# aelefebv/nellie

Hardware: AMD Instinct MI355X
Metric: Mvoxel/s multiscale Frangi (5 sigma) + Label, float32, frame resident in HBM (higher is better)
Workload: dtype f32; 1 GPU; synthetic 1024x1024x1024 float32 volume (N(100,5) noise + Gaussian tube segments, seed 2345), 0.1 um isotropic, 5-scale Frangi + Label, full hot path per step, frame resident in HBM; voxels=1073741824, labels=265, one_pass_scales=5, fast_div_proven=2, hessian_tile_rows=16

## Files before the change

nellie_amd/csrc/label_runs.inc:

```

struct RunRec { int row; unsigned int x; };
struct RunN { const unsigned int *p; i64 h; i64 cap; };
__device__ __forceinline__ i64 run_n(const RunN &r) { const i64 n = r.p ? (i64)*r.p : r.h; return n > r.cap ? 0 : n; }

__device__ __forceinline__ unsigned long long rl_word(const unsigned long long *__restrict__ bits, i64 row, int w, int wpr,
                                                      int nx, bool invert) {
    unsigned long long v = bits[row * wpr + w];
    if (invert) v = ~v;
    const int rem = nx - w * 64;
    if (rem < 64) v &= (rem <= 0) ? 0ull : ((1ull << rem) - 1ull);
    return v;
}

__global__ void __launch_bounds__(256)
rl_threshold_pack_kernel(const float *__restrict__ f, const unsigned long long *__restrict__ support, unsigned long long *__restrict__ bits,
                         int has_thr, float thr_host, int nx, i64 nrows, int wpr, const float *__restrict__ thr_dev = nullptr) {
    const float thr = thr_dev ? *thr_dev : thr_host;
    const i64 wstride = ((i64)gridDim.x * blockDim.x) >> 6;
    const int lane = threadIdx.x & 63;
    const bool row_words = support && wpr <= 64;
    const i64 first = ((i64)blockIdx.x * blockDim.x + threadIdx.x) >> 6;
    unsigned long long mine_next = (row_words && first < nrows && lane < wpr) ? support[first * wpr + lane] : 0ull;
    unsigned long long st_res = 0ull;
    i64 st_row = -1;
// ... 433 lines not shown
        const i64 i = base + k;
        if (i >= nruns) break;
        const int root = parent[i];
        const int len = (int)(runs[i].x >> 16) - (int)(runs[i].x & 0xffffu);
        unsigned int h = ((unsigned int)root * 2654435761u) >> 24;
        bool done = false;
        for (int probe = 0; probe < 8 && !done; ++probe) {
            const int old = atomicCAS(&keys[h], -1, root);
            if (old == -1 || old == root) { atomicAdd(&vals[h], len); done = true; }
            else h = (h + 1) & (RL_HT - 1);
        }
        if (!done) atomicAdd(&area[root], len);
    }
    __syncthreads();
    for (int k = threadIdx.x; k < RL_HT; k += 256)
        if (keys[k] >= 0 && vals[k]) atomicAdd(&area[keys[k]], vals[k]);
  }
}

__global__ void __launch_bounds__(256)
rl_keep_kernel(const RunRec *__restrict__ runs, const int *__restrict__ parent, const int *__restrict__ area, int min_area,
               unsigned long long *__restrict__ bits, RunN rn, int wpr) {
    const i64 nruns = run_n(rn);
    for (i64 i = (i64)blockIdx.x * blockDim.x + threadIdx.x; i < nruns; i += (i64)gridDim.x * blockDim.x) {
        if (area[parent[i]] < min_area) continue;
        const RunRec r = runs[i];
        rl_set_bits(bits, r.row, wpr, (int)(r.x & 0xffffu), (int)(r.x >> 16));
    }
}

__global__ void __launch_bounds__(256)
majority_bits_kernel(const unsigned long long *__restrict__ in, unsigned long long *__restrict__ out, VolGeom v, int wpr, i64 z_lo, i64 z_hi) {
    const unsigned int ny = (unsigned int)v.ny, uw = (unsigned int)wpr;
    const unsigned int nw = (unsigned int)(z_hi - z_lo) * ny * uw;
    const unsigned int t0 = blockIdx.x * blockDim.x + threadIdx.x;
    if (t0 >= nw) return;
    const unsigned int w = t0 % uw, row0 = t0 / uw;
    const int y = (int)(row0 % ny), z = (int)(row0 / ny) + (int)z_lo;
    const i64 t = ((i64)z * ny + y) * wpr + w;
    const bool last = (w == uw - 1u);
    const unsigned long long top = 1ull << (((int)v.nx - 1) & 63);
    const unsigned long long valid = (top << 1) - 1ull;
    unsigned long long c0 = 0, c1 = 0, c2 = 0, c3 = 0, c4 = 0;
    auto add = [&](unsigned long long b) {
        unsigned long long t0_ = c0 & b; c0 ^= b; b = t0_;
        t0_ = c1 & b; c1 ^= b; b = t0_;
        t0_ = c2 & b; c2 ^= b; b = t0_;
        t0_ = c3 & b; c3 ^= b; b = t0_;
        c4 ^= b;
    };
    unsigned long long cw[9];
    i64 rws[9];
    unsigned long long any = 0ull;
#pragma unroll
    for (int dz = -1; dz <= 1; ++dz) {
        int zz = z + dz;
        const i64 gg = v.gz0 + zz;
        if (gg < 0 || gg >= v.gnz) zz = z;
#pragma unroll
        for (int dy = -1; dy <= 1; ++dy) {
            int yy = y + dy;
            yy = yy < 0 ? 0 : (yy >= (int)ny ? (int)ny - 1 : yy);
            const int k = (dz + 1) * 3 + (dy + 1);
            rws[k] = ((i64)zz * ny + yy) * wpr;
            cw[k] = in[rws[k] + w];
            any |= cw[k];
        }
    }
    if (any == 0ull) { out[t] = 0ull; return; }
#pragma unroll
    for (int k = 0; k < 9; ++k) {
        const unsigned long long cur = cw[k];
        const unsigned long long prev = (w > 0u) ? in[rws[k] + w - 1] : 0ull;
        const unsigned long long left = (cur << 1) | ((w > 0u) ? (prev >> 63) : (cur & 1ull));
        const unsigned long long next = last ? 0ull : in[rws[k] + w + 1];
        const unsigned long long right = (cur >> 1) | (last ? (cur & top) : (next << 63));
        add(left); add(cur); add(right);
    }
    unsigned long long res = c4 | (c3 & c2 & c1);
    if (last) res &= valid;
    out[t] = res;
}

__global__ void __launch_bounds__(256)
rl_paint_kernel(const unsigned long long *__restrict__ bits, const unsigned int *__restrict__ row_off, const int *__restrict__ parent,
                const int *__restrict__ newid, int *__restrict__ out, i64 row0, i64 row1, int wpr, int nx) {
    const i64 wstride = ((i64)gridDim.x * blockDim.x) >> 6;
    const int lane = threadIdx.x & 63;
    for (i64 row = row0 + (((i64)blockIdx.x * blockDim.x + threadIdx.x) >> 6); row < row1; row += wstride) {
        const unsigned int seen0 = row_off[row], nr = row_off[row + 1] - seen0;
        unsigned int seen = seen0;
        int *orow = out + (row - row0) * nx;
        const bool vec = ((nx & 3) == 0) && ((reinterpret_cast<size_t>(orow) & 15) == 0);
        if (nr == 0u && vec) {
            for (int q = lane; q < nx / 4; q += 64) reinterpret_cast<int4 *>(orow)[q] = make_int4(0, 0, 0, 0);
            continue;
        }
        const int lab_mine = ((unsigned int)lane < nr) ? newid[parent[seen0 + lane]] : 0;
        if (vec) {
            for (int q = lane; q < nx / 4; q += 64) reinterpret_cast<int4 *>(orow)[q] = make_int4(0, 0, 0, 0);
            asm volatile("s_waitcnt vmcnt(0)" ::: "memory");
            unsigned long long carry = 0;
            int prev_w = -2;
            for (int wb = 0; wb < wpr; wb += 64) {
                const unsigned long long mine = (wb + lane < wpr) ? rl_word(bits, row, wb + lane, wpr, nx, false) : 0ull;
                unsigned long long todo = __ballot(mine != 0ull);
                while (todo) {
                    const int wl = __builtin_ctzll(todo);
                    todo &= todo - 1;
                    const int w = wb + wl;
                    const unsigned long long v = __shfl(mine, wl, 64);
                    if (w != prev_w + 1) carry = 0ull;
                    const unsigned long long starts = v & ~((v << 1) | carry);
                    const int x = w * 64 + lane;
                    const bool set = (v >> lane) & 1ull;
                    const unsigned long long below = starts & ((lane == 63) ? ~0ull : ((1ull << (lane + 1)) - 1ull));
                    const unsigned int rl = set ? (seen - seen0) + (unsigned int)__builtin_popcountll(below) - 1u : 0u;
                    int lab = __shfl(lab_mine, (int)(rl & 63u), 64);
                    if (set && rl >= 64u) lab = newid[parent[seen0 + rl]];
                    if (set && x < nx) orow[x] = lab;
                    seen += (unsigned int)__builtin_popcountll(starts);
                    carry = v >> 63;
                    prev_w = w;
                }
            }
            continue;
        }
        unsigned long long carry = 0;
        for (int wb = 0; wb < wpr; wb += 64) {
            const unsigned long long mine = (wb + lane < wpr) ? rl_word(bits, row, wb + lane, wpr, nx, false) : 0ull;
            const int wend = wpr - wb < 64 ? wpr - wb : 64;
            for (int wl = 0; wl < wend; ++wl) {
                const int w = wb + wl;
                const unsigned long long v = __shfl(mine, wl, 64);
                const unsigned long long starts = v & ~((v << 1) | carry);
                const int x = w * 64 + lane;
                const bool set = (v >> lane) & 1ull;
                const unsigned long long below = starts & ((lane == 63) ? ~0ull : ((1ull << (lane + 1)) - 1ull));
                const unsigned int rl = set ? (seen - seen0) + (unsigned int)__builtin_popcountll(below) - 1u : 0u;
                int lab = __shfl(lab_mine, (int)(rl & 63u), 64);
                if (set && rl >= 64u) lab = newid[parent[seen0 + rl]];
                if (x < nx) orow[x] = set ? lab : 0;
                seen += (unsigned int)__builtin_popcountll(starts);
                carry = v >> 63;
            }
        }
    }
}

#define SL_FILL 0
#define SL_AREA 1
#define SL_NUMBER 2

__global__ void __launch_bounds__(256)
sl_first_own_kernel(const RunRec *__restrict__ runs, const int *__restrict__ parent, int *__restrict__ aux, i64 nruns, int row_lo, int row_hi,
                    const unsigned int *__restrict__ own_first_ptr) {
    const i64 i = (i64)blockIdx.x * blockDim.x + threadIdx.x;
    if (i >= nruns) return;
    const int own_first = (int)*own_first_ptr;
    const int row = runs[i].row;
    if (row < row_lo || row >= row_hi) return;
    const int r = parent[i];
    if (r >= own_first) { if (r == (int)i) aux[i] = (int)i; return; }
    if ((int)i < __hip_atomic_load(&aux[r], __ATOMIC_RELAXED, __HIP_MEMORY_SCOPE_AGENT)) atomicMin(&aux[r], (int)i);
}
__global__ void __launch_bounds__(256)
sl_area_kernel(const RunRec *__restrict__ runs, const int *__restrict__ parent, int *__restrict__ area, i64 nruns, int row_lo, int row_hi) {
    __shared__ int keys[RL_HT];
    __shared__ int vals[RL_HT];
    for (int k = threadIdx.x; k < RL_HT; k += 256) { keys[k] = -1; vals[k] = 0; }
    __syncthreads();
    const i64 base = (i64)blockIdx.x * RL_CHUNK;
    for (int k = threadIdx.x; k < RL_CHUNK; k += 256) {
        const i64 i = base + k;
        if (i >= nruns) break;
        const RunRec r = runs[i];
        if (r.row < row_lo || r.row >= row_hi) continue;
        const int root = parent[i];
        const int len = (int)(r.x >> 16) - (int)(r.x & 0xffffu);
        unsigned int h = ((unsigned int)root * 2654435761u) >> 24;
        bool done = false;
        for (int probe = 0; probe < 8 && !done; ++probe) {
            const int old = atomicCAS(&keys[h], -1, root);
            if (old == -1 || old == root) { atomicAdd(&vals[h], len); done = true; }
            else h = (h + 1) & (RL_HT - 1);
        }
        if (!done) atomicAdd(&area[root], len);
    }
    __syncthreads();
    for (int k = threadIdx.x; k < RL_HT; k += 256)
        if (keys[k] >= 0 && vals[k]) atomicAdd(&area[keys[k]], vals[k]);
}
struct SlabPlanes { int row[4]; };
__global__ void __launch_bounds__(1024)
sl_boundary_kernel(const unsigned int *__restrict__ row_off, const int *__restrict__ proot, SlabPlanes pl, int ny, int capE,
                   int *__restrict__ bidx, int *__restrict__ hdr) {
    __shared__ unsigned int s_w[16];
    __shared__ unsigned int s_base;
    const int p = blockIdx.x;
    if (pl.row[p] < 0) { if (threadIdx.x == 0) hdr[p] = 0; return; }
    const unsigned int r0 = row_off[pl.row[p]], r1 = row_off[pl.row[p] + ny];
    const int lane = threadIdx.x & 63, w = threadIdx.x >> 6;
    if (threadIdx.x == 0) s_base = 0;
    __syncthreads();
    for (unsigned int c0 = r0; c0 < r1; c0 += 1024) {
        const unsigned int i = c0 + threadIdx.x;
        const bool f = i < r1 && (!proot || proot[i] == (int)i);
        const unsigned long long b = __ballot(f);
        const unsigned int below = (unsigned int)__builtin_popcountll(b & ((1ull << lane) - 1ull));
        if (lane == 0) s_w[w] = (unsigned int)__builtin_popcountll(b);
        __syncthreads();
        unsigned int off = s_base;
        for (int q = 0; q < w; ++q) off += s_w[q];
        if (f && off + below < (unsigned int)capE) bidx[(size_t)p * capE + off + below] = (int)i;
        __syncthreads();
        if (threadIdx.x == 0) { unsigned int t = 0; for (int q = 0; q < 16; ++q) t += s_w[q]; s_base += t; }
        __syncthreads();
    }
    if (threadIdx.x == 0) hdr[p] = (int)s_base;
}
__global__ void __launch_bounds__(256)
sl_table2_kernel(const int *__restrict__ parent, const int *__restrict__ aux, const uint8_t *__restrict__ flag, const int *__restrict__ bidx,
                 int capE, const int *__restrict__ hdr, int *__restrict__ blob, const unsigned int *__restrict__ nruns_ptr) {
    const int p = blockIdx.x;
    int cnt[4], total = 0, off = 8, over = 0;
// ... 63 lines not shown
```

nellie_amd/csrc/nellie_hip.hip:

```cpp
#include "nl_host.h"

struct RcclApi {
    void *handle = nullptr;
    decltype(&ncclGetUniqueId) GetUniqueId = nullptr;
    decltype(&ncclCommInitRank) CommInitRank = nullptr;
    decltype(&ncclCommDestroy) CommDestroy = nullptr;
    decltype(&ncclGetErrorString) GetErrorString = nullptr;
    decltype(&ncclGroupStart) GroupStart = nullptr;
    decltype(&ncclGroupEnd) GroupEnd = nullptr;
    decltype(&ncclSend) Send = nullptr;
    decltype(&ncclRecv) Recv = nullptr;
    decltype(&ncclAllReduce) AllReduce = nullptr;
    decltype(&ncclBroadcast) Broadcast = nullptr;
    decltype(&ncclAllGather) AllGather = nullptr;
    bool ok = false;
};
static RcclApi &rccl_real() {
    static RcclApi api;
    if (!api.handle) {
        std::string rp;
        if (const char *e = getenv("ROCM_PATH")) rp = std::string(e) + "/lib/librccl.so.1";
        const char *names[] = {rp.c_str(), "/opt/rocm/lib/librccl.so.1", "/opt/rocm/lib/librccl.so", "librccl.so.1", "librccl.so"};
        for (const char *n : names) { if (!*n) continue; api.handle = dlopen(n, RTLD_NOW | RTLD_GLOBAL); if (api.handle) break; }
        if (api.handle) {
// ... 327 lines not shown
    if (ok) ok = alloc((void **)&c->d_rows, ((size_t)nzl * ny + 2) * 2 * 4);
    if (ok) ok = alloc(&c->d_small, 1 << 16);
    c->vq_chunks = (int)vq_chunks(nzl, ny, nx);
    {
        const size_t qe = (size_t)vq_alloc_entries(nzl, ny, nx);
        if (ok) ok = alloc((void **)&c->d_vq, qe * 32);
        if (ok) ok = alloc((void **)&c->d_vq_count, (size_t)vq_alloc_regions(nzl, ny, nx) * 4);
        c->spec_ok = vq_spec_entries(nzl, ny, nx) > 0;
    }
    c->blk_cap = (n + SCAN_CHUNK - 1) / SCAN_CHUNK + 1;
    if (ok) ok = alloc(&c->d_blk, (size_t)c->blk_cap * 4);
    if (ok && hipHostMalloc(&c->h_small, 1 << 16, hipHostMallocDefault) != hipSuccess) {
        rc = nl_fail(err, errlen, NL_ENOMEM, "hipHostMalloc failed [out of memory]"); ok = false;
    }
    int side_prio = -1;
    { const char *e = getenv("NELLIE_SIDE_PRIO"); if (e) side_prio = atoi(e); }
    int prio_lo = 0, prio_hi = 0;
    (void)hipDeviceGetStreamPriorityRange(&prio_lo, &prio_hi);
    const int side_p = side_prio < 0 ? prio_hi : (side_prio > 0 ? prio_lo : (prio_lo + prio_hi) / 2);
    if (ok && (hipStreamCreateWithPriority(&c->side, hipStreamNonBlocking, side_p) != hipSuccess ||
               hipEventCreateWithFlags(&c->ev_side, hipEventDisableTiming) != hipSuccess ||
               hipEventCreateWithFlags(&c->ev_main, hipEventDisableTiming) != hipSuccess ||
               hipEventCreateWithFlags(&c->ev_ahead, hipEventDisableTiming) != hipSuccess)) {
        rc = nl_fail(err, errlen, NL_EHIP, "stream/event creation failed"); ok = false;
    }
    if (ok && (hipStreamCreateWithFlags(&c->stream, hipStreamNonBlocking) != hipSuccess ||
               hipEventCreate(&c->t0) != hipSuccess || hipEventCreate(&c->t1) != hipSuccess)) {
        rc = nl_fail(err, errlen, NL_EHIP, "stream/event creation failed"); ok = false;
    }
    if (!ok) { nl_ctx_destroy(c); return rc; }
    *out = c;
    return NL_OK;
}

extern "C" int nl_sync(nl_ctx *c, char *err, size_t errlen) {
    if (!c) return nl_fail(err, errlen, NL_EINVAL, "ctx is NULL");
    NL_HIP(hipSetDevice(c->device));
    NL_HIP(hipStreamSynchronize(c->stream));
    NL_HIP(hipStreamSynchronize(c->side));
    if (c->xstream) NL_HIP(hipStreamSynchronize(c->xstream));
    return NL_OK;
}


int upload_convert(nl_ctx *c, const void *host, int dtype, float *dst, i64 count, char *err, size_t errlen) {
    const size_t es = dtype_size(dtype);
    if (!es) return nl_fail(err, errlen, NL_EINVAL, "unsupported dtype code %d", dtype);
    if (dtype == NL_F32) {
        NL_HIP(hipMemcpyAsync(dst, host, (size_t)count * 4, hipMemcpyHostToDevice, c->stream));
        NL_HIP(hipStreamSynchronize(c->stream));
        return NL_OK;
    }
    void *raw = nullptr;
    bool own = false;
    for (int k = 0; k < 4 && !raw; ++k) {
        const bool contains = (dst >= c->f[k] && dst < c->f[k] + c->n);
        if (!contains && k != c->i_vmax && es <= 4) raw = c->f[k];
    }
    if (!raw) { NL_HIP(hipMalloc(&raw, (size_t)count * es)); own = true; }
    NL_HIP(hipMemcpyAsync(raw, host, (size_t)count * es, hipMemcpyHostToDevice, c->stream));
    const unsigned int g = grid1d(count);
    switch (dtype) {
        case NL_U8: convert_kernel<uint8_t><<<g, 256, 0, c->stream>>>((const uint8_t *)raw, dst, count); break;
        case NL_I8: convert_kernel<int8_t><<<g, 256, 0, c->stream>>>((const int8_t *)raw, dst, count); break;
        case NL_U16: convert_kernel<uint16_t><<<g, 256, 0, c->stream>>>((const uint16_t *)raw, dst, count); break;
        case NL_I16: convert_kernel<int16_t><<<g, 256, 0, c->stream>>>((const int16_t *)raw, dst, count); break;
        case NL_U32: convert_kernel<uint32_t><<<g, 256, 0, c->stream>>>((const uint32_t *)raw, dst, count); break;
        case NL_I32: convert_kernel<int32_t><<<g, 256, 0, c->stream>>>((const int32_t *)raw, dst, count); break;
        case NL_F64: convert_kernel<double><<<g, 256, 0, c->stream>>>((const double *)raw, dst, count); break;
        case NL_U64: convert_kernel<uint64_t><<<g, 256, 0, c->stream>>>((const uint64_t *)raw, dst, count); break;
        case NL_I64: convert_kernel<int64_t><<<g, 256, 0, c->stream>>>((const int64_t *)raw, dst, count); break;
    }
    NL_CHECK_LAUNCH();
    NL_HIP(hipStreamSynchronize(c->stream));
    if (own) hipFree(raw);
    return NL_OK;
}

extern "C" int nl_filter_load(nl_ctx *c, const void *host, int dtype, int64_t z0, int64_t z1, char *err, size_t errlen) {
    NL_ENTER(c);
    NL_JOIN_SIDE(c);
    if (!host || z0 < 0 || z1 > c->nzl || z0 >= z1) return nl_fail(err, errlen, NL_EINVAL, "bad plane range [%lld,%lld)", (i64)z0, (i64)z1);
    c->i_gauss = 0; c->i_vmax = 3; c->i_labels = -1; c->frangi_ready = 0;
    c->gauss_ext = nullptr;
    if (c->ahead_pending) NL_HIP(hipStreamWaitEvent(c->stream, c->ev_ahead, 0));
    c->ahead_pending = 0;
    c->fsq_cache_valid = 0;
    NL_HIP(zero_small((char *)c->d_small + (52 << 10), 4, c->stream));
    c->vmax_zero_lo = c->vmax_zero_hi = 0;
    const i64 plane = c->ny * c->nx;
    int rc = upload_convert(c, host, dtype, c->f[0] + z0 * plane, (z1 - z0) * plane, err, errlen);
    if (rc) return rc;
    c->mask_slots_used = 0;
    NL_HIP(hipStreamSynchronize(c->stream));
    return NL_OK;
}

extern "C" int nl_input_load(nl_ctx *c, const void *host, int dtype, int64_t z0, int64_t z1, char *err, size_t errlen) {
    NL_ENTER(c);
    const size_t es = dtype_size(dtype);
    if (!es) return nl_fail(err, errlen, NL_EINVAL, "unsupported dtype code %d", dtype);
    if (!host || z0 < 0 || z1 > c->nzl || z0 >= z1) return nl_fail(err, errlen, NL_EINVAL, "bad plane range [%lld,%lld)", (i64)z0, (i64)z1);
    if (c->d_input && c->input_borrowed) { c->d_input = nullptr; c->input_borrowed = 0; }
    if (c->d_input && c->input_dtype != dtype) { hipFree(c->d_input); c->d_input = nullptr; }
    if (!c->d_input) NL_HIP(hipMalloc(&c->d_input, (size_t)c->n * es));
    c->input_dtype = dtype;
    const i64 plane = c->ny * c->nx;
    NL_HIP(hipMemcpyAsync((char *)c->d_input + (size_t)z0 * plane * es, host, (size_t)(z1 - z0) * plane * es, hipMemcpyHostToDevice, c->stream));
    NL_HIP(hipStreamSynchronize(c->stream));
    return NL_OK;
}

extern "C" int nl_filter_begin(nl_ctx *c, char *err, size_t errlen) {
    NL_ENTER(c);
    NL_JOIN_SIDE(c);
    if (!c->d_input) return nl_fail(err, errlen, NL_ESTATE, "nl_filter_begin before nl_input_load");
    c->i_gauss = 0; c->i_vmax = 3; c->i_labels = -1; c->frangi_ready = 0;
    c->mask_slots_used = 0;
    c->gauss_ext = nullptr;
    if (c->ahead_pending) NL_HIP(hipStreamWaitEvent(c->stream, c->ev_ahead, 0));
    c->ahead_pending = 0;
    c->fsq_cache_valid = 0;
    NL_HIP(zero_small((char *)c->d_small + (52 << 10), 4, c->stream));
    c->vmax_zero_lo = c->vmax_zero_hi = 0;
    if (c->input_dtype == NL_F32 && !getenv("NELLIE_COPY_INPUT")) {
        c->gauss_ext = (float *)c->d_input;
        return NL_OK;
    }
    ProfScope ps(c, "load");
    const unsigned int g = grid1d(c->n);
    switch (c->input_dtype) {
        case NL_U8: convert_kernel<uint8_t><<<g, 256, 0, c->stream>>>((const uint8_t *)c->d_input, c->f[0], c->n); break;
        case NL_I8: convert_kernel<int8_t><<<g, 256, 0, c->stream>>>((const int8_t *)c->d_input, c->f[0], c->n); break;
        case NL_U16: convert_kernel<uint16_t><<<g, 256, 0, c->stream>>>((const uint16_t *)c->d_input, c->f[0], c->n); break;
        case NL_I16: convert_kernel<int16_t><<<g, 256, 0, c->stream>>>((const int16_t *)c->d_input, c->f[0], c->n); break;
        case NL_U32: convert_kernel<uint32_t><<<g, 256, 0, c->stream>>>((const uint32_t *)c->d_input, c->f[0], c->n); break;
        case NL_I32: convert_kernel<int32_t><<<g, 256, 0, c->stream>>>((const int32_t *)c->d_input, c->f[0], c->n); break;
        case NL_F32: convert_kernel<float><<<g, 256, 0, c->stream>>>((const float *)c->d_input, c->f[0], c->n); break;
        case NL_F64: convert_kernel<double><<<g, 256, 0, c->stream>>>((const double *)c->d_input, c->f[0], c->n); break;
        case NL_U64: convert_kernel<uint64_t><<<g, 256, 0, c->stream>>>((const uint64_t *)c->d_input, c->f[0], c->n); break;
        case NL_I64: convert_kernel<int64_t><<<g, 256, 0, c->stream>>>((const int64_t *)c->d_input, c->f[0], c->n); break;
    }
    NL_CHECK_LAUNCH();
    c->mask_slots_used = 0;
    return NL_OK;
}


static bool gauss_can_yx(const nl_ctx *c, const double *wy, int ry, const double *wx, int rx) {
    return wy && wx && ry == rx && ry >= 1 && ry <= GM_MAX_R && ry <= c->ny && !getenv("NELLIE_NO_FUSED_YX");
}
static int gauss_step_volumes(const nl_ctx *c, const double *wz, const double *wy, int ry, const double *wx, int rx) {
    return (wz ? 1 : 0) + (gauss_can_yx(c, wy, ry, wx, rx) ? 1 : (wy ? 1 : 0) + (wx ? 1 : 0));
}

extern "C" int nl_gauss_step(nl_ctx *c, const double *wz, int rz, const double *wy, int ry, const double *wx, int rx,
                             int64_t z0, int64_t z1, char *err, size_t errlen) {
    NL_ENTER(c);
    if (c->ahead_pending) return nl_fail(err, errlen, NL_ESTATE, "nl_gauss_step while a step enqueued ahead is uncommitted");
    if (z0 < 0 || z1 > c->nzl || z0 >= z1) return nl_fail(err, errlen, NL_EINVAL, "bad plane range [%lld,%lld)", (i64)z0, (i64)z1);
    if (c->halo_pending) {
        ProfScope ps(c, "halo_wait");
        NL_HIP(hipStreamWaitEvent(c->stream, c->ev_x_done, 0));
        c->halo_pending = 0;
    }
    const VolGeom v = geom(c);
    const dim3 grid((unsigned)((c->nx + 255) / 256), (unsigned)c->ny, (unsigned)(z1 - z0));
    int src = c->i_gauss;
    const float *srcp = gauss_cur(c);
    GaussW gw;
    int rc;
    const bool can_yx = gauss_can_yx(c, wy, ry, wx, rx);
    bool fused_yx = false;
    const char *e_fz = getenv("NELLIE_GAUSS_FUSED");
    const bool fused_zyx = e_fz ? atoi(e_fz) != 0 : c->n >= ((i64)1 << 26);
    if (fused_zyx && wz && can_yx && gyx_tiled() && gl_zyx_ok(c, rz, ry, c->f[(src + 1) % 3]) &&
        memcmp(wy, wx, (size_t)(2 * ry + 1) * sizeof(double)) == 0) {
        GaussW gy;
        if ((rc = fill_gw(gw, wz, rz, err, errlen)) || (rc = fill_gw(gy, wy, ry, err, errlen))) return rc;
        if ((z0 - rz < 0 && c->gz0 > 0) || (z1 - 1 + rz >= c->nzl && c->gz0 + c->nzl < c->gnz))
            return nl_fail(err, errlen, NL_EINVAL, "Z pass of radius %d on planes [%lld,%lld) reaches outside the local slab", rz, (i64)z0, (i64)z1);
        const int dst = (src + 1) % 3;
        char scope[32];
        snprintf(scope, sizeof scope, "gauss_zyx<%d,%d>", rz, ry);
        ProfScope ps(c, scope);
        static int zero_in_passing = -1;
        if (zero_in_passing < 0) { const char *e = getenv("NELLIE_ZERO_IN_GAUSS"); zero_in_passing = (e && !atoi(e)) ? 0 : 1; }
        const bool zero = zero_in_passing && c->mask_slots_used == 0 && c->vmax_zero_hi == 0 && c->stream != c->side;
        (void)gl_zyx(c, rz, ry, srcp, c->f[dst], v, z0, z1, gauss_ws_of(gw), gauss_ws_of(gy), zero ? c->f[c->i_vmax] : nullptr);
        if (zero) { c->vmax_zero_lo = z0; c->vmax_zero_hi = z1; }
        NL_CHECK_LAUNCH();
        src = dst; srcp = c->f[dst];
        fused_yx = true;
        wz = nullptr;
    }
    if (wz) {
        if ((rc = fill_gw(gw, wz, rz, err, errlen))) return rc;
        if ((z0 - rz < 0 && c->gz0 > 0) || (z1 - 1 + rz >= c->nzl && c->gz0 + c->nzl < c->gnz))
            return nl_fail(err, errlen, NL_EINVAL, "Z pass of radius %d on planes [%lld,%lld) reaches outside the local slab", rz, (i64)z0, (i64)z1);
        const int dst = (src + 1) % 3;
        ProfScope ps(c, "gauss_z");
        if (!gl_fast(0, c, srcp, c->f[dst], v, z0, z1, gw)) gl_axis(0, false, c, grid, srcp, c->f[dst], v, z0, z1, gw);
        NL_CHECK_LAUNCH();
        src = dst; srcp = c->f[dst];
    }
    if (!fused_yx && can_yx) {
        GaussW gy, gx;
        if ((rc = fill_gw(gy, wy, ry, err, errlen))) return rc;
        if ((rc = fill_gw(gx, wx, rx, err, errlen))) return rc;
        const GaussWS wsy = gauss_ws_of(gy), wsx = gauss_ws_of(gx);
        const int dst = (src + 1) % 3;
        ProfScope ps(c, "gauss_yx");
        const dim3 g2((unsigned)((c->nx + GYX_COLS - 1) / GYX_COLS), (unsigned)((c->ny + v.chunk - 1) / v.chunk), (unsigned)(z1 - z0));
        (void)gl_yx(c, gyx_tiled(), false, ry, srcp, c->f[dst], v, z0, z1, wsy, wsx, g2);
        NL_CHECK_LAUNCH();
        src = dst; srcp = c->f[dst];
        fused_yx = true;
    }
    if (wy && !fused_yx) {
        if ((rc = fill_gw(gw, wy, ry, err, errlen))) return rc;
        const int dst = (src + 1) % 3;
        ProfScope ps(c, "gauss_y");
        if (!gl_fast(1, c, srcp, c->f[dst], v, z0, z1, gw)) gl_axis(1, false, c, grid, srcp, c->f[dst], v, z0, z1, gw);
        NL_CHECK_LAUNCH();
        src = dst; srcp = c->f[dst];
    }
    if (wx && !fused_yx) {
        if ((rc = fill_gw(gw, wx, rx, err, errlen))) return rc;
        const int dst = (src + 1) % 3;
        ProfScope ps(c, "gauss_x");
        if (!gl_fast(2, c, srcp, c->f[dst], v, z0, z1, gw)) gl_axis(2, false, c, grid, srcp, c->f[dst], v, z0, z1, gw);
        NL_CHECK_LAUNCH();
        src = dst; srcp = c->f[dst];
    }
    c->i_gauss = src;
    c->fsq_cache_valid = 0;
    if (srcp != c->gauss_ext) c->gauss_ext = nullptr;
    return NL_OK;
}

extern "C" int nl_gauss_step_ahead(nl_ctx *c, const double *wz, int rz, const double *wy, int ry, const double *wx, int rx,
                                   int64_t z0, int64_t z1, char *err, size_t errlen) {
    NL_ENTER(c);
    if (c->ahead_pending) return nl_fail(err, errlen, NL_ESTATE, "a step enqueued ahead is already pending");
    if (gauss_step_volumes(c, wz, wy, ry, wx, rx) > 2)
        return nl_fail(err, errlen, NL_ESTATE, "a cascade step of three passes (radii %d / %d / %d) cannot run ahead: it needs the current Gaussian's volume", rz, ry, rx);
    NL_HIP(hipEventRecord(c->ev_main, c->stream));
    hipStream_t ahead_stream = c->side;
    NL_HIP(hipStreamWaitEvent(ahead_stream, c->ev_main, 0));
    const int cur_idx = c->i_gauss;
    float *cur_ext = c->gauss_ext;
    hipStream_t main_stream = c->stream;
    c->stream = ahead_stream;
    const int rc = nl_gauss_step(c, wz, rz, wy, ry, wx, rx, z0, z1, err, errlen);
    c->stream = main_stream;
    if (rc) { c->i_gauss = cur_idx; c->gauss_ext = cur_ext; return rc; }
    c->ahead_gauss = c->i_gauss;
    c->i_gauss = cur_idx; c->gauss_ext = cur_ext;
    NL_HIP(hipEventRecord(c->ev_ahead, ahead_stream));
    c->ahead_pending = 1;
    return NL_OK;
}

extern "C" int nl_gauss_commit(nl_ctx *c, char *err, size_t errlen) {
    NL_ENTER(c);
    if (!c->ahead_pending) return nl_fail(err, errlen, NL_ESTATE, "nl_gauss_commit without nl_gauss_step_ahead");
    NL_HIP(hipStreamWaitEvent(c->stream, c->ev_ahead, 0));
    c->i_gauss = c->ahead_gauss;
    c->gauss_ext = nullptr;
    c->ahead_pending = 0;
    c->fsq_cache_valid = 0;
    return NL_OK;
}

static int make_lattice(const nl_ctx *c, i64 sz, i64 sy, i64 sx, Lattice &L, char *err, size_t errlen) {
    if (sz < 1 || sy < 1 || sx < 1) return nl_fail(err, errlen, NL_EINVAL, "strides must be >= 1");
    L.sz = sz; L.sy = sy; L.sx = sx;
    const i64 g_lo = c->gz0 + c->own_lo, g_hi = c->gz0 + c->own_hi;
    const i64 k_lo = (g_lo + sz - 1) / sz, k_hi = (g_hi + sz - 1) / sz;
    L.cz = k_hi > k_lo ? k_hi - k_lo : 0;
    L.zfirst = k_lo * sz - c->gz0;
    L.cy = (c->ny + sy - 1) / sy;
    L.cx = (c->nx + sx - 1) / sx;
    return NL_OK;
}

static int make_field(nl_ctx *c, int field, FieldSrc &fs, char *err, size_t errlen) {
    fs.field = field; fs.hp = hessp(c); fs.max_abs = c->frob_max_abs; fs.max_finite = c->frob_max_finite;
    fs.two_d = c->two_d; fs.bits = nullptr; fs.wpr = 0; fs.fsq_cache = nullptr; fs.norm_dev = nullptr;
    if (field == NL_FIELD_GAUSS) fs.p = gauss_cur(c);
    else if (field == NL_FIELD_FROB) {
        if (!c->have_spacing) return nl_fail(err, errlen, NL_ESTATE, "NL_FIELD_FROB before nl_hessian_stats");
        fs.p = gauss_cur(c);
    } else if (field == NL_FIELD_FRANGI) fs.p = c->f[c->i_vmax];
    else if (field == NL_FIELD_VESSELNESS) {
        if (c->mask_slots_used == 0) return nl_fail(err, errlen, NL_ESTATE, "NL_FIELD_VESSELNESS before any scale was evaluated");
        NL_JOIN_SIDE(c);
        fs.p = c->f[c->i_vmax];
        fs.wpr = (int)((c->nx + 63) / 64);
        fs.bits = (const unsigned long long *)c->m[0] + (i64)((c->mask_slots_used - 1) & 1) * (c->nzl * c->ny * fs.wpr);
    } else return nl_fail(err, errlen, NL_EINVAL, "unknown field %d", field);
    return NL_OK;
}

static int use_fsq_cache(nl_ctx *c, FieldSrc &fs, const Lattice &L, char *err, size_t errlen) {
    if (fs.field != NL_FIELD_FROB) return NL_OK;
    const i64 total = L.cz * L.cy * L.cx;
    if (total == 0) return NL_OK;
    if (!(c->fsq_cache_valid && c->fsq_cache_key[0] == L.sz && c->fsq_cache_key[1] == L.sy && c->fsq_cache_key[2] == L.sx)) {
        if (total > c->fsq_cache_cap) {
            if (c->d_fsq_cache) NL_HIP(hipFree(c->d_fsq_cache));
            c->d_fsq_cache = nullptr; c->fsq_cache_cap = 0;
            NL_HIP(hipMalloc((void **)&c->d_fsq_cache, (size_t)total * 4));
            c->fsq_cache_cap = total;
        }
        ProfScope ps(c, "sample");
        sample_fsq_kernel<<<(unsigned)((total + 255) / 256), 256, 0, c->stream>>>(fs, geom(c), L, c->d_fsq_cache);
        NL_CHECK_LAUNCH();
        c->fsq_cache_key[0] = L.sz; c->fsq_cache_key[1] = L.sy; c->fsq_cache_key[2] = L.sx;
        c->fsq_cache_valid = 1;
    }
    fs.fsq_cache = c->d_fsq_cache;
    return NL_OK;
}

extern "C" int nl_sample_gather(nl_ctx *c, int field, int64_t sz, int64_t sy, int64_t sx, float *out, int64_t cap,
                                int64_t *n, char *err, size_t errlen) {
    NL_ENTER(c);
    Lattice L; FieldSrc fs; int rc;
    if ((rc = make_lattice(c, sz, sy, sx, L, err, errlen))) return rc;
    if ((rc = make_field(c, field, fs, err, errlen))) return rc;
    if ((rc = use_fsq_cache(c, fs, L, err, errlen))) return rc;
    const i64 total = L.cz * L.cy * L.cx;
    if (n) *n = total;
    if (total == 0 || (!out && cap == 0)) return NL_OK;
    if (!out || cap < total) return nl_fail(err, errlen, NL_EINVAL, "output capacity %lld < %lld samples", (i64)cap, total);
    float *stage = c->f[(c->i_gauss + 1) % 3];
    if (total > c->n) return nl_fail(err, errlen, NL_EINVAL, "lattice larger than the volume");
    {
        ProfScope ps(c, "sample");
        sample_gather_kernel<<<(unsigned)((total + 255) / 256), 256, 0, c->stream>>>(fs, geom(c), L, stage);
        NL_CHECK_LAUNCH();
    }
    NL_HIP(hipMemcpyAsync(out, stage, (size_t)total * 4, hipMemcpyDeviceToHost, c->stream));
    NL_HIP(hipStreamSynchronize(c->stream));
    return NL_OK;
}

// ... 631 lines not shown
    { int rc = resolve_enqueue(c, vp, d_cnt, nullptr, err, errlen); if (rc) return rc; }
    *hit = 1;
    if (mask_count) {
        int rcc = nl_vesselness_count(c, mask_count, err, errlen);
        if (rcc) return rcc;
    }
    return NL_OK;
}


static void host_edges(float first, float last, int nbins, float *edges) {
    if (first == last) { first = first - 0.5f; last = last + 0.5f; }
    volatile float delta = last - first;
    const float div = (float)nbins;
    volatile float step = delta / div;
    for (int i = 0; i <= nbins; ++i) {
        volatile float y = (float)i;
        if (step == 0.0f) { y = y / div; y = y * delta; } else y = y * step;
        y = y + first;
        edges[i] = (i == nbins) ? last : y;
    }
}
static inline unsigned int f2u(float x) { unsigned int u; memcpy(&u, &x, 4); return u; }
static inline float u2f(unsigned int u) { float x; memcpy(&x, &u, 4); return x; }
static inline float py_min_f(float a, float b) { return b < a ? b : a; }

static int chain_verify(const ChainScale &s, double division, double margin, double test_scale) {
    if (s.flags) return s.flags;
    int bad = 0;
    double tri, otsu; int st;
    {
        hist_thresholds_host<float>((const int64_t *)s.h_gauss.counts, s.h_gauss.edges, NL_CHAIN_BINS, &tri, &otsu, &st);
        const float g = py_min_f((float)tri, (float)otsu);
        const float gamma = g > 0.0f ? g : 1.1920929e-07f;
        const float gamma_sq = (float)(2.0 * std::pow((double)gamma, 2.0));
        if (st || f2u(gamma) != f2u(s.gamma) || f2u(gamma_sq) != f2u(s.gamma_sq)) bad = 1;
        float e[NL_CHAIN_BINS + 1];
        host_edges(u2f(s.h_gauss.res[0]), u2f(s.h_gauss.res[1]), NL_CHAIN_BINS, e);
        if (memcmp(e, s.h_gauss.edges, sizeof(e))) bad = 1;
    }
    {
        hist_thresholds_host<float>((const int64_t *)s.h_raw.counts, s.h_raw.edges, NL_CHAIN_BINS, &tri, &otsu, &st);
        const double t = (double)py_min_f((float)tri, (float)otsu) * test_scale / division;
        const float lo = (float)(t * t * (1.0 - margin)), hi = (float)(t * t * (1.0 + margin));
        if (st || f2u(lo) != f2u(s.fsq_lo) || f2u(hi) != f2u(s.fsq_hi)) bad = 1;
        float e[NL_CHAIN_BINS + 1];
        host_edges(u2f(s.h_raw.res[0]), u2f(s.h_raw.res[1]), NL_CHAIN_BINS, e);
        if (memcmp(e, s.h_raw.edges, sizeof(e))) bad = 1;
    }
    {
        const float max_abs32 = u2f(s.stats[0]), max_fsq32 = u2f(s.stats[1]);
        const float max_abs = max_abs32 <= 0.0f ? 1.0f : max_abs32;
        volatile float mf = sqrtf(max_fsq32); mf = mf / max_abs;
        volatile float mn = u2f(s.h_raw.res[0]) / max_abs, mx = u2f(s.h_raw.res[1]) / max_abs;
        if (f2u(max_abs) != f2u(s.max_abs) || f2u((float)mf) != f2u(s.max_frob) || f2u((float)mn) != f2u(s.nmn) || f2u((float)mx) != f2u(s.nmx) ||
            f2u(s.norm[0]) != f2u(max_abs) || s.norm[1] != 0.0f) bad = 1;
        float e[NL_CHAIN_BINS + 1];
        host_edges((float)mn, (float)mx, NL_CHAIN_BINS, e);
        if (memcmp(e, s.h_exact.edges, sizeof(e))) bad = 1;
        hist_thresholds_host<float>((const int64_t *)s.h_exact.counts, s.h_exact.edges, NL_CHAIN_BINS, &tri, &otsu, &st);
        const float thr = py_min_f((float)tri, (float)otsu);
        const float thr_cmp = (float)((double)thr / division);
        const float fsq_min = mask_threshold_on_fsq(max_abs, 1, thr_cmp);
        if (st || f2u(thr) != f2u(s.thr) || f2u(thr_cmp) != f2u(s.thr_cmp) || f2u(fsq_min) != f2u(s.fsq_min) || s.m_inf != ((0.0f > thr_cmp) ? 1 : 0)) bad = 1;
        if (!(fsq_min >= s.fsq_lo && fsq_min <= s.fsq_hi) || !((float)mf > thr_cmp)) bad = 1;
    }
    return bad ? NL_CF_VERIFY : 0;
}

extern "C" int nl_chain_begin(nl_ctx *c, int n_scales, char *err, size_t errlen) {
    NL_ENTER(c);
    if (n_scales < 1 || n_scales > NL_CHAIN_MAX_SCALES) return nl_fail(err, errlen, NL_EINVAL, "a chain holds 1..%d scales", NL_CHAIN_MAX_SCALES);
    if (!c->two_d && (!c->spec_ok || !hv_rs(c))) return nl_fail(err, errlen, NL_ESTATE, "the device-resident chain needs the 3-D one-pass walk");
    if (!c->d_chain) {
        NL_HIP(hipMalloc(&c->d_chain, sizeof(ChainScale) * NL_CHAIN_MAX_SCALES));
        NL_HIP(hipHostMalloc(&c->h_chain, sizeof(ChainScale) * NL_CHAIN_MAX_SCALES, hipHostMallocDefault));
        NL_HIP(hipEventCreateWithFlags(&c->ev_chain, hipEventDisableTiming));
    }
    chain_init_kernel<<<16, 256, 0, c->stream>>>((ChainScale *)c->d_chain, n_scales);
    chain_init2_kernel<<<1, 64, 0, c->stream>>>((ChainScale *)c->d_chain, n_scales);
    NL_CHECK_LAUNCH();
    c->chain_n = n_scales; c->chain_k = 0; c->chain_copy_pending = 0;
    c->def_resolve = 0;
    return NL_OK;
}

extern "C" int nl_chain_scale(nl_ctx *c, const double spacing[3], int64_t sz, int64_t sy, int64_t sx, double alpha_sq, double beta_sq,
                              double division, double margin, double test_scale, int64_t z0, int64_t z1, char *err, size_t errlen) {
    NL_ENTER(c);
    if (!c->d_chain || c->chain_k >= c->chain_n) return nl_fail(err, errlen, NL_ESTATE, "nl_chain_scale outside nl_chain_begin .. nl_chain_finish");
    if (!(division != 0.0)) return nl_fail(err, errlen, NL_EINVAL, "the chain needs a non-zero threshold division");
    int rc;
    if ((rc = set_spacing(c, spacing, err, errlen))) return rc;
    if ((rc = resolve_deferred_launch(c, true, err, errlen))) return rc;
    ChainScale *cs = (ChainScale *)c->d_chain + c->chain_k;
    c->chain_par[c->chain_k][0] = division; c->chain_par[c->chain_k][1] = margin; c->chain_par[c->chain_k][2] = test_scale;
    ++c->chain_k;
    c->frob_max_abs = 1.0f; c->frob_max_finite = 0.0f;
    if (c->two_d) {
        if (!chain_unfused_sampling()) {
            if ((rc = range_hist_pair_enqueue(c, sz, sy, sx, NL_CHAIN_BINS, (char *)&cs->h_gauss, (char *)&cs->h_raw, nullptr, nullptr, err, errlen))) return rc;
        } else {
            if ((rc = range_hist_enqueue_at(c, NL_FIELD_GAUSS, sz, sy, sx, NL_CHAIN_BINS, (char *)&cs->h_gauss, nullptr, err, errlen))) return rc;
            if ((rc = range_hist_enqueue_at(c, NL_FIELD_FROB, sz, sy, sx, NL_CHAIN_BINS, (char *)&cs->h_raw, nullptr, err, errlen))) return rc;
        }
        chain_thr1_kernel<<<2, 64, 0, c->stream>>>(cs, division, margin, test_scale);
        {
            ProfScope ps(c, "hessian_stats");
            hessian2d_stats_kernel<<<grid2d_rows(c->nx, c->ny), 256, 0, c->stream>>>(gauss_cur(c), geom(c), hessp(c), cs->stats);
        }
        chain_post_kernel<<<1, 64, 0, c->stream>>>(cs);
        NL_CHECK_LAUNCH();
        {
            Lattice L; FieldSrc fs;
            if ((rc = make_lattice(c, sz, sy, sx, L, err, errlen))) return rc;
            if ((rc = make_field(c, NL_FIELD_FROB, fs, err, errlen))) return rc;
            if ((rc = use_fsq_cache(c, fs, L, err, errlen))) return rc;
            fs.norm_dev = cs->norm;
            const i64 total = L.cz * L.cy * L.cx;
            ProfScope ps(c, "sample");
            sample_edges_kernel<<<1, 64, 0, c->stream>>>(cs->h_exact.res, NL_CHAIN_BINS, cs->h_exact.edges, cs->h_exact.res + 4);
            const size_t sh = (size_t)(NL_CHAIN_BINS + 2) * 4 + (size_t)NL_CHAIN_BINS * 4;
            if (total > 0) sample_hist_kernel<<<grid1d(total, 256, sample_grid_cap()), 256, sh, c->stream>>>(fs, geom(c), L, cs->h_exact.edges, NL_CHAIN_BINS, cs->h_exact.counts, cs->h_exact.res + 4);
            NL_CHECK_LAUNCH();
        }
        chain_thr2_kernel<<<1, 64, 0, c->stream>>>(cs, division);
        NL_CHECK_LAUNCH();
        VessP vp{};
        vp.alpha_sq = (float)alpha_sq; vp.beta_sq = (float)beta_sq; vp.use_thr = 1;
        vp.cnt_lo = (int)c->own_lo; vp.cnt_hi = (int)c->own_hi;
        vp.first = c->mask_slots_used == 0 ? 1 : 0;
        vp.nan_flag = (unsigned int *)((char *)c->d_small + NL_NAN_FLAG_OFF);
        ProfScope ps(c, "vesselness");
        const int wpr = (int)((c->nx + 63) / 64);
        const i64 slot_words = c->nzl * c->ny * wpr;
        const int k_scale = c->mask_slots_used++;
        vp.have_prev = k_scale > 0;
        unsigned long long *cm = (unsigned long long *)c->m[0] + (i64)(k_scale & 1) * slot_words;
        const unsigned long long *pm = (unsigned long long *)c->m[0] + (i64)((k_scale + 1) & 1) * slot_words;
        if (vp.first && !vmax_is_zero(c, 0, c->nzl)) NL_HIP(hipMemsetAsync(c->f[c->i_vmax], 0, (size_t)c->n * 4, c->stream));
        c->vmax_zero_hi = 0;
        c->spec_valid = 0;
        vesselness2d_kernel<<<grid2d_rows((i64)wpr * 64, c->ny), 256, 0, c->stream>>>(gauss_cur(c), c->f[c->i_vmax], cm, pm, wpr, geom(c), hessp(c), vp,
                                                                                        &cs->cnt_resolve, (const float *)cs);
        NL_CHECK_LAUNCH();
        return NL_OK;
    }
    if (!chain_unfused_sampling()) {
        if ((rc = range_hist_pair_enqueue(c, sz, sy, sx, NL_CHAIN_BINS, (char *)&cs->h_gauss, (char *)&cs->h_raw, nullptr, nullptr, err, errlen))) return rc;
    } else {
        if ((rc = range_hist_enqueue_at(c, NL_FIELD_GAUSS, sz, sy, sx, NL_CHAIN_BINS, (char *)&cs->h_gauss, nullptr, err, errlen))) return rc;
        if ((rc = range_hist_enqueue_at(c, NL_FIELD_FROB, sz, sy, sx, NL_CHAIN_BINS, (char *)&cs->h_raw, nullptr, err, errlen))) return rc;
    }
    chain_thr1_kernel<<<2, 64, 0, c->stream>>>(cs, division, margin, test_scale);
    NL_CHECK_LAUNCH();
    if ((rc = spec_enqueue(c, spacing, 0.0f, 0.0f, z0, z1, cs->stats, &cs->cnt_walk, &cs->fsq_lo, err, errlen))) return rc;
    const bool defer = resolve_defer_ok(c) && c->fsq_cache_valid;
    hipStream_t st = c->stream;
    chain_post_kernel<<<1, 64, 0, st>>>(cs);
    NL_CHECK_LAUNCH();
    {
        Lattice L; FieldSrc fs;
        if ((rc = make_lattice(c, sz, sy, sx, L, err, errlen))) return rc;
        if ((rc = make_field(c, NL_FIELD_FROB, fs, err, errlen))) return rc;
        if ((rc = use_fsq_cache(c, fs, L, err, errlen))) return rc;
        fs.norm_dev = cs->norm;
        const i64 total = L.cz * L.cy * L.cx;
        ProfScope ps(c, "sample", st);
        sample_edges_kernel<<<1, 64, 0, st>>>(cs->h_exact.res, NL_CHAIN_BINS, cs->h_exact.edges, cs->h_exact.res + 4);
        const size_t sh = (size_t)(NL_CHAIN_BINS + 2) * 4 + (size_t)NL_CHAIN_BINS * 4;
        if (total > 0) sample_hist_kernel<<<grid1d(total, 256, sample_grid_cap()), 256, sh, st>>>(fs, geom(c), L, cs->h_exact.edges, NL_CHAIN_BINS, cs->h_exact.counts, cs->h_exact.res + 4);
        NL_CHECK_LAUNCH();
        if (fused(c) && (rc = reduce_u64_sum(c, cs->h_exact.counts, NL_CHAIN_BINS, err, errlen))) return rc;
    }
    chain_thr2_kernel<<<1, 64, 0, st>>>(cs, division);
    NL_CHECK_LAUNCH();
    VessP vp{};
    vp.alpha_sq = (float)alpha_sq; vp.beta_sq = (float)beta_sq; vp.use_thr = 1;
    vp.cnt_lo = (int)c->own_lo; vp.cnt_hi = (int)c->own_hi;
    vp.first = c->mask_slots_used == 0 ? 1 : 0;
    if (defer) {
        memcpy(c->def_vp, &vp, sizeof(VessP));
        c->def_cnt = &cs->cnt_resolve; c->def_params = (const float *)cs; c->def_resolve = 1;
        return NL_OK;
    }
    return resolve_enqueue(c, vp, &cs->cnt_resolve, (const float *)cs, err, errlen);
}

extern "C" int nl_chain_flush(nl_ctx *c, char *err, size_t errlen) {
    NL_ENTER(c);
    if (!c->d_chain || c->chain_k < 1) return nl_fail(err, errlen, NL_ESTATE, "nl_chain_flush without scales");
    { int rcd = resolve_deferred_launch(c, false, err, errlen); if (rcd) return rcd; }
    NL_JOIN_SIDE(c);
    NL_HIP(hipMemcpyAsync(c->h_chain, c->d_chain, sizeof(ChainScale) * (size_t)c->chain_k, hipMemcpyDeviceToHost, c->stream));
    NL_HIP(hipEventRecord(c->ev_chain, c->stream));
    c->chain_copy_pending = 1;
    return NL_OK;
}

extern "C" int nl_chain_finish(nl_ctx *c, int *flags, double *gamma, double *max_abs, double *thr, int64_t *mask_count, char *err, size_t errlen) {
    NL_ENTER(c);
    if (!c->d_chain || c->chain_k < 1) return nl_fail(err, errlen, NL_ESTATE, "nl_chain_finish without scales");
    const int n = c->chain_k;
    if (!c->chain_copy_pending) { int rcd = resolve_deferred_launch(c, false, err, errlen); if (rcd) return rcd; }
    if (c->chain_copy_pending) {
        NL_HIP(hipEventSynchronize(c->ev_chain));
        c->chain_copy_pending = 0;
    } else {
        NL_JOIN_SIDE(c);
        NL_HIP(hipMemcpyAsync(c->h_chain, c->d_chain, sizeof(ChainScale) * (size_t)n, hipMemcpyDeviceToHost, c->stream));
        NL_HIP(hipStreamSynchronize(c->stream));
    }
    const ChainScale *h = (const ChainScale *)c->h_chain;
    for (int k = 0; k < n; ++k) {
        const int f = chain_verify(h[k], c->chain_par[k][0], c->chain_par[k][1], c->chain_par[k][2]);
        if (flags) flags[k] = f;
        if (gamma) gamma[k] = (double)h[k].gamma;
        if (max_abs) max_abs[k] = (double)h[k].max_abs;
        if (thr) thr[k] = (double)h[k].thr;
        if (mask_count) mask_count[k] = (int64_t)(h[k].cnt_walk + h[k].cnt_resolve);
    }
    c->chain_n = 0;
    return NL_OK;
}

extern "C" int nl_chain_log(nl_ctx *c, int k, int which, int64_t *counts, float *edges, float *range, double *scalars, char *err, size_t errlen) {
    if (!c || !c->h_chain || k < 0 || k >= NL_CHAIN_MAX_SCALES || which < 0 || which > 2) return nl_fail(err, errlen, NL_EINVAL, "bad chain log request");
    const ChainScale &s = ((const ChainScale *)c->h_chain)[k];
    const ChainHist &h = which == 0 ? s.h_gauss : (which == 1 ? s.h_raw : s.h_exact);
    if (counts) memcpy(counts, h.counts, sizeof(h.counts));
    if (edges) memcpy(edges, h.edges, sizeof(h.edges));
    if (range) { range[0] = u2f(h.res[0]); range[1] = u2f(h.res[1]); }
    if (scalars) {
        scalars[0] = s.fsq_lo; scalars[1] = s.fsq_hi; scalars[2] = s.gamma_sq; scalars[3] = s.fsq_min; scalars[4] = s.thr_cmp; scalars[5] = s.max_frob;
        scalars[6] = s.tri[which]; scalars[7] = s.otsu[which];
    }
    return NL_OK;
}

extern "C" int nl_vesselness_step(nl_ctx *c, float gamma_sq, float alpha_sq, float beta_sq, int use_thr, float thr,
                                  int64_t z0, int64_t z1, int64_t *mask_count, char *err, size_t errlen) {
    NL_ENTER(c);
    if (z0 < 0 && z1 < 0) { z0 = c->own_lo; z1 = c->own_hi; }
    if (z0 < 0 || z1 > c->nzl || z0 >= z1) return nl_fail(err, errlen, NL_EINVAL, "bad plane range [%lld,%lld)", (i64)z0, (i64)z1);
    if (!c->have_spacing) return nl_fail(err, errlen, NL_ESTATE, "nl_vesselness_step before nl_hessian_stats");
    NL_JOIN_SIDE(c);
    unsigned long long *d_cnt = (unsigned long long *)c->d_small;
    NL_HIP(zero_small(d_cnt, 8, c->stream));
    VessP vp = make_vessp(c, gamma_sq, alpha_sq, beta_sq, use_thr, thr);
    vp.qcap = HM_REGION;
    c->spec_valid = 0;
    if (c->two_d) {
        ProfScope ps(c, "vesselness");
        const int wpr = (int)((c->nx + 63) / 64);
        const i64 slot_words = c->nzl * c->ny * wpr;
        const int k_scale = c->mask_slots_used++;
        vp.have_prev = k_scale > 0;
        unsigned long long *cm = (unsigned long long *)c->m[0] + (i64)(k_scale & 1) * slot_words;
        const unsigned long long *pm = (unsigned long long *)c->m[0] + (i64)((k_scale + 1) & 1) * slot_words;
        if (vp.first && !vmax_is_zero(c, 0, c->nzl)) NL_HIP(hipMemsetAsync(c->f[c->i_vmax], 0, (size_t)c->n * 4, c->stream));
        c->vmax_zero_hi = 0;
        vesselness2d_kernel<<<grid2d_rows((i64)wpr * 64, c->ny), 256, 0, c->stream>>>(gauss_cur(c), c->f[c->i_vmax], cm, pm, wpr, geom(c), hessp(c), vp, d_cnt);
        NL_CHECK_LAUNCH();
    } else {
        ProfScope ps(c, "vesselness");
        const int ntx = (int)((c->nx + HM_TX - 1) / HM_TX);
        const int wpr = (int)((c->nx + 63) / 64);
        const i64 slot_words = c->nzl * c->ny * wpr;
        const int k_scale = c->mask_slots_used++;
        vp.have_prev = k_scale > 0;
        unsigned long long *cm = (unsigned long long *)c->m[0] + (i64)(k_scale & 1) * slot_words;
        const unsigned long long *pm = (unsigned long long *)c->m[0] + (i64)((k_scale + 1) & 1) * slot_words;
        const i64 plane = c->ny * c->nx;
        const i64 planes_per_launch = (i64)c->vq_chunks * HM_ZCHUNK;
        const VQueue vq{(float4 *)c->d_vq, c->d_vq_count};
        if (vp.first && !vmax_is_zero(c, z0, z1))
            NL_HIP(hipMemsetAsync(c->f[c->i_vmax] + z0 * plane, 0, (size_t)(z1 - z0) * plane * 4, c->stream));
        c->vmax_zero_hi = 0;
        const int rs = hv_rs(c);
        const int ty = rs ? 2 * rs : hm_ty();
        const int nty = (int)((c->ny + ty - 1) / ty);
        if (rs) vp.qcap = 2 * hv_np(c) * HM_REGION;
#define NL_LAUNCH_VESS(TYV, FASTV, HR)                                                                                    \
        hessian_g_kernel<1, TYV, FASTV><<<nblocks, HGCfg<TYV>::NT, HGCfg<TYV>::lds_bytes(), c->stream>>>(                 \
            gauss_cur(c), cm, pm, wpr, geom(c), HR, vp, vq, (int)za, (int)zb, ntx, nty, nullptr, d_cnt)
        for (i64 za = z0; za < z1; za += planes_per_launch) {
            const i64 zb = za + planes_per_launch < z1 ? za + planes_per_launch : z1;
            const int nzc = (int)((zb - za + HM_ZCHUNK - 1) / HM_ZCHUNK);
            const unsigned nblocks = (unsigned)(ntx * nty * nzc);
            if (rs) NL_HIP(nl_hv_launch(HvLaunch{1, rs, hv_np(c), hv_fastv(c), nblocks, c->stream, gauss_cur(c), cm, pm, wpr, geom(c), hessp(c), vp, vq, (int)za, (int)zb,
                                                 ntx, nty, nullptr, d_cnt, nullptr}));
            else if (ty == 8) { if (c->fast_div) NL_LAUNCH_VESS(8, true, hessdv_fast(c)); else NL_LAUNCH_VESS(8, false, hessdv_exact(c)); }
            else { if (c->fast_div) NL_LAUNCH_VESS(16, true, hessdv_fast(c)); else NL_LAUNCH_VESS(16, false, hessdv_exact(c)); }
            NL_CHECK_LAUNCH();
            const unsigned nregions = nblocks * (unsigned)(rs ? rs / hv_np(c) : ty);
            vesselness_queue_kernel<false><<<resolve_grid((nregions + 3) / 4), 256, 0, c->stream>>>(vq.ent, vq.count, nregions, c->f[c->i_vmax], za * plane, vp,
                                                                                      nullptr, nullptr, wpr, (int)c->ny, (int)c->nx, za, nullptr, nullptr);
            NL_CHECK_LAUNCH();
        }
#undef NL_LAUNCH_VESS
        NL_CHECK_LAUNCH();
    }
    if (mask_count) {
        NL_HIP(hipMemcpyAsync(c->h_small, d_cnt, 8, hipMemcpyDeviceToHost, c->stream));
        NL_HIP(hipStreamSynchronize(c->stream));
// ... 76 lines not shown
    if (z0 < 0 && z1 < 0) { z0 = c->own_lo; z1 = c->own_hi; }
    if (z0 < 0 || z1 > c->nzl || z0 >= z1) return nl_fail(err, errlen, NL_EINVAL, "bad plane range [%lld,%lld)", (i64)z0, (i64)z1);
    NL_JOIN_SIDE(c);
    unsigned long long *d_cnt = (unsigned long long *)c->d_small;
    NL_HIP(zero_small(d_cnt, 8, c->stream));
    const i64 plane = c->ny * c->nx;
    if (c->mask_slots_used == 0 && !vmax_is_zero(c, z0, z1))
        NL_HIP(hipMemsetAsync(c->f[c->i_vmax] + z0 * plane, 0, (size_t)(z1 - z0) * plane * 4, c->stream));
    c->vmax_zero_hi = 0;
    {
        ProfScope ps(c, "finish");
        const int wpr = (int)((c->nx + 63) / 64);
        const i64 quads = (z1 - z0) * c->ny * ((c->nx + 3) / 4);
        const i64 slot_words = c->nzl * c->ny * wpr;
        const int last = c->mask_slots_used > 0 ? ((c->mask_slots_used - 1) & 1) : 0;
        finish_kernel<<<grid1d(quads, 256, 256 * 16), 256, 0, c->stream>>>(c->f[c->i_vmax], (const unsigned long long *)c->m[0] + last * slot_words,
                                                               c->mask_slots_used > 0 ? 1 : 0, slot_words, wpr, geom(c), z0, z1, c->own_lo, c->own_hi, d_cnt);
        NL_CHECK_LAUNCH();
    }
    NL_HIP(hipMemcpyAsync(c->h_small, d_cnt, 8, hipMemcpyDeviceToHost, c->stream));
    NL_HIP(hipStreamSynchronize(c->stream));
    if (n_positive) *n_positive = (int64_t)(*(unsigned long long *)c->h_small);
    c->frangi_ready = 1;
    return NL_OK;
}

extern "C" int nl_remove_edges(nl_ctx *c, int margin, int64_t *n_positive, char *err, size_t errlen) {
    NL_ENTER(c);
    NL_JOIN_SIDE(c);
    if (!c->frangi_ready) return nl_fail(err, errlen, NL_ESTATE, "nl_remove_edges before a Frangi frame exists");
    if (margin < 0) return nl_fail(err, errlen, NL_EINVAL, "margin %d is negative", margin);
    unsigned long long *d_cnt = (unsigned long long *)c->d_small;
    NL_HIP(zero_small(d_cnt, 8, c->stream));
    {
        ProfScope ps(c, "finish");
        const i64 r0 = c->own_lo - 2 > 0 ? c->own_lo - 2 : 0, r1 = c->own_hi + 2 < c->nzl ? c->own_hi + 2 : c->nzl;
        remove_edges_kernel<<<(unsigned)(r1 - r0), 256, 0, c->stream>>>(c->f[c->i_vmax], geom(c), r0, margin, c->own_lo, c->own_hi, d_cnt);
        NL_CHECK_LAUNCH();
    }
    NL_HIP(hipMemcpyAsync(c->h_small, d_cnt, 8, hipMemcpyDeviceToHost, c->stream));
    NL_HIP(hipStreamSynchronize(c->stream));
    if (n_positive) *n_positive = (int64_t)(*(unsigned long long *)c->h_small);
    return NL_OK;
}

static int mask_volume_enqueue(nl_ctx *c, float thr, const float *thr_dev, int *dst_out, char *err, size_t errlen) {
    int dst = -1;
    for (int k = 0; k < 3; ++k) if (k != c->i_gauss) { dst = k; break; }
    *dst_out = dst;
    ProfScope ps(c, "mask_volume");
    const int wpr = (int)((c->nx + 63) / 64);
    const VolGeom v = geom(c);
    const i64 m0 = c->own_lo - 2 > 0 ? c->own_lo - 2 : 0, m1 = c->own_hi + 2 < c->nzl ? c->own_hi + 2 : c->nzl;
    const i64 e0 = c->own_lo - 1 > 0 ? c->own_lo - 1 : 0, e1 = c->own_hi + 1 < c->nzl ? c->own_hi + 1 : c->nzl;
    unsigned long long *bM = (unsigned long long *)c->m[1], *bE = (unsigned long long *)c->m[2], *bD = (unsigned long long *)c->m[0];
    nl_launch_threshold_pack(grid1d((m1 - m0) * c->ny * 64, 256, (i64)1 << 22), c->stream,
        c->f[c->i_vmax] + m0 * c->ny * c->nx, nullptr, bM + m0 * c->ny * wpr, 1, thr, (int)c->nx, (m1 - m0) * c->ny, wpr, thr_dev);
    NL_CHECK_LAUNCH();
    bits_morph6_kernel<0><<<(unsigned)(((e1 - e0) * c->ny * wpr + 255) / 256), 256, 0, c->stream>>>(bM, bE, v, wpr, e0, e1, c->two_d);
    NL_CHECK_LAUNCH();
    bits_morph6_kernel<1><<<(unsigned)(((c->own_hi - c->own_lo) * c->ny * wpr + 255) / 256), 256, 0, c->stream>>>(bE, bD, v, wpr, c->own_lo, c->own_hi, c->two_d);
    NL_CHECK_LAUNCH();
    apply_bits_kernel<<<grid1d((c->own_hi - c->own_lo) * c->ny * ((c->nx + 3) / 4), 256, 256 * 32), 256, 0, c->stream>>>(
        c->f[c->i_vmax], bD, c->f[dst], v, wpr, c->own_lo, c->own_hi);
    NL_CHECK_LAUNCH();
    return NL_OK;
}
static void mask_volume_commit(nl_ctx *c, int dst) {
    float *tmp = c->f[c->i_vmax];
    c->f[c->i_vmax] = c->f[dst];
    c->f[dst] = tmp;
}

extern "C" int nl_mask_volume(nl_ctx *c, float thr, char *err, size_t errlen) {
    NL_ENTER(c);
    int dst, rc;
    if ((rc = mask_volume_enqueue(c, thr, nullptr, &dst, err, errlen))) return rc;
    mask_volume_commit(c, dst);
    return NL_OK;
}

static int mask_volume_fused_enqueue(nl_ctx *c, float thr, const float *thr_dev, unsigned long long *d_cnt, int *dst_out, char *err, size_t errlen) {
    int dst = -1;
    for (int k = 0; k < 3; ++k) if (k != c->i_gauss) { dst = k; break; }
    *dst_out = dst;
    NL_HIP(zero_small(d_cnt, 8, c->stream));
    ProfScope ps(c, "mask_volume");
    const int wpr = (int)((c->nx + 63) / 64);
    const VolGeom v = geom(c);
    const i64 slot_words = c->nzl * c->ny * wpr;
    const int last = (c->mask_slots_used - 1) & 1;
    const unsigned long long *alive = (const unsigned long long *)c->m[0] + (i64)last * slot_words;
    const i64 m0 = c->own_lo - 2 > 0 ? c->own_lo - 2 : 0, m1 = c->own_hi + 2 < c->nzl ? c->own_hi + 2 : c->nzl;
    const i64 e0 = c->own_lo - 1 > 0 ? c->own_lo - 1 : 0, e1 = c->own_hi + 1 < c->nzl ? c->own_hi + 1 : c->nzl;
    unsigned long long *bM = (unsigned long long *)c->m[1], *bE = (unsigned long long *)c->m[2];
    unsigned long long *bD = (unsigned long long *)c->m[0] + (i64)(last ^ 1) * slot_words;
    pack_masked_kernel<<<grid1d((m1 - m0) * c->ny * 64, 256, 256 * 16), 256, 0, c->stream>>>(
        c->f[c->i_vmax], alive, bM, thr, thr_dev, (int)c->nx, m0 * c->ny, m1 * c->ny, wpr, c->own_lo * c->ny, c->own_hi * c->ny, d_cnt);
    NL_CHECK_LAUNCH();
    bits_morph6_kernel<0><<<(unsigned)(((e1 - e0) * c->ny * wpr + 255) / 256), 256, 0, c->stream>>>(bM, bE, v, wpr, e0, e1, c->two_d);
    NL_CHECK_LAUNCH();
    bits_morph6_kernel<1><<<(unsigned)(((c->own_hi - c->own_lo) * c->ny * wpr + 255) / 256), 256, 0, c->stream>>>(bE, bD, v, wpr, c->own_lo, c->own_hi, c->two_d);
    NL_CHECK_LAUNCH();
    apply_bits_pos_kernel<<<grid1d(((c->own_hi - c->own_lo) * c->ny + APPLY_ROWS - 1) / APPLY_ROWS * 64, 256, (i64)1 << 22), 256, 0, c->stream>>>(
        c->f[c->i_vmax], bD, c->f[dst], v, wpr, c->own_lo, c->own_hi);
    NL_CHECK_LAUNCH();
    if (fused(c)) NL_NCCL(rccl().AllReduce(d_cnt, d_cnt, 1, ncclUint64, ncclSum, (ncclComm_t)c->comm, c->stream));
    return NL_OK;
}
static void mask_volume_fused_commit(nl_ctx *c, int dst) {
    float *tmp = c->f[c->i_vmax];
    c->f[c->i_vmax] = c->f[dst];
    c->f[dst] = tmp;
    c->frangi_ready = 1;
    c->d_support = (const unsigned long long *)c->m[0] + (i64)(((c->mask_slots_used - 1) & 1) ^ 1) * (c->nzl * c->ny * (i64)((c->nx + 63) / 64));
    c->support_epoch = c->epoch.load();
}

extern "C" int nl_mask_volume_fused(nl_ctx *c, float thr, int64_t *n_positive, char *err, size_t errlen) {
    NL_ENTER(c);
    if (c->mask_slots_used == 0) return nl_fail(err, errlen, NL_ESTATE, "nl_mask_volume_fused before any scale was evaluated");
    NL_JOIN_SIDE(c);
    unsigned long long *d_cnt = (unsigned long long *)c->d_small;
    int dst, rc;
    if ((rc = mask_volume_fused_enqueue(c, thr, nullptr, d_cnt, &dst, err, errlen))) return rc;
    NL_HIP(hipMemcpyAsync(c->h_small, d_cnt, 8, hipMemcpyDeviceToHost, c->stream));
    NL_HIP(hipStreamSynchronize(c->stream));
    if (n_positive) *n_positive = (int64_t)(*(unsigned long long *)c->h_small);
    mask_volume_fused_commit(c, dst);
    return NL_OK;
}

static int pct_buffers(nl_ctx *c, char *err, size_t errlen) {
    if (!c->d_pct) {
        NL_HIP(hipMalloc(&c->d_pct, 128 + (size_t)2 * PCT_BINS * 4));
        NL_HIP(hipHostMalloc(&c->h_pct, 128, hipHostMallocDefault));
    }
    return NL_OK;
}
static int pct_enqueue(nl_ctx *c, const float *samples, const unsigned int *d_n, i64 max_n, float q, char *err, size_t errlen) {
    PctRec *rec = (PctRec *)c->d_pct;
    unsigned int *hist = (unsigned int *)((char *)c->d_pct + 128);
    NL_HIP(hipMemcpyAsync(&rec->n, d_n, 4, hipMemcpyDeviceToDevice, c->stream));
    NL_HIP(hipMemcpyAsync(&rec->n_local, d_n, 4, hipMemcpyDeviceToDevice, c->stream));
    if (fused(c)) NL_NCCL(rccl().AllReduce(&rec->n, &rec->n, 1, ncclUint32, ncclSum, (ncclComm_t)c->comm, c->stream));
    ProfScope ps(c, "sample");
    pct_begin_kernel<<<1, 64, 0, c->stream>>>(rec, q);
    const unsigned grid = grid1d(max_n > 0 ? max_n : 1, 256, 256 * 256);
#define NL_PCT_LEVEL(L)                                                                                            \
    NL_HIP(hipMemsetAsync(hist, 0, (size_t)2 * PCT_BINS * 4, c->stream));                                           \
    pct_hist_kernel<L><<<grid, 256, 0, c->stream>>>(samples, d_n, rec, hist);                                       \
    if (fused(c)) NL_NCCL(rccl().AllReduce(hist, hist, (size_t)2 * PCT_BINS, ncclUint32, ncclSum, (ncclComm_t)c->comm, c->stream)); \
    pct_select_kernel<L><<<1, 256, 0, c->stream>>>(rec, hist);
    NL_PCT_LEVEL(0) NL_PCT_LEVEL(1) NL_PCT_LEVEL(2)
#undef NL_PCT_LEVEL
    NL_CHECK_LAUNCH();
    return NL_OK;
}

extern "C" int nl_tail_enqueue(nl_ctx *c, int64_t sz, int64_t sy, int64_t sx, double q, char *err, size_t errlen) {
    NL_ENTER(c);
    if (c->mask_slots_used == 0) return nl_fail(err, errlen, NL_ESTATE, "nl_tail_enqueue before any scale was evaluated");
    if (c->two_d) return nl_fail(err, errlen, NL_EINVAL, "nl_tail_enqueue is the 3-D epilogue");
    int rc;
    if ((rc = pct_buffers(c, err, errlen))) return rc;
    Lattice L; FieldSrc fs;
    if ((rc = make_lattice(c, sz, sy, sx, L, err, errlen))) return rc;
    if ((rc = make_field(c, NL_FIELD_VESSELNESS, fs, err, errlen))) return rc;
    const i64 total = L.cz * L.cy * L.cx;
    if (total > c->n) return nl_fail(err, errlen, NL_EINVAL, "lattice larger than the volume");
    float *stage = c->f[(c->i_gauss + 1) % 3];
    if (stage == c->f[c->i_vmax]) return nl_fail(err, errlen, NL_ESTATE, "no free volume for the samples");
    unsigned int *d_n = (unsigned int *)((char *)c->d_pct + 64);
    unsigned long long *d_cnt = (unsigned long long *)((char *)c->d_pct + 72);
    NL_HIP(zero_small(d_n, 4, c->stream));
    if (total > 0) {
        ProfScope ps(c, "sample");
        sample_gather_pos_kernel<<<(unsigned)((total + 255) / 256), 256, 0, c->stream>>>(fs, geom(c), L, stage, d_n);
        NL_CHECK_LAUNCH();
    }
    if ((rc = pct_enqueue(c, stage, d_n, total, (float)q, err, errlen))) return rc;
    int dst;
    if ((rc = mask_volume_fused_enqueue(c, 0.0f, &((PctRec *)c->d_pct)->thr, d_cnt, &dst, err, errlen))) return rc;
    NL_HIP(hipMemcpyAsync(c->h_pct, c->d_pct, 80, hipMemcpyDeviceToHost, c->stream));
    c->tail_pending = 1; c->tail_dst = dst;
    return NL_OK;
}

extern "C" int nl_tail_finish(nl_ctx *c, int commit, int64_t *n_samples, float *a, float *b, float *gamma, float *thr, int64_t *n_positive,
                              char *err, size_t errlen) {
    NL_ENTER(c);
    if (!c->tail_pending) return nl_fail(err, errlen, NL_ESTATE, "nl_tail_finish without nl_tail_enqueue");
    NL_HIP(hipStreamSynchronize(c->stream));
    c->tail_pending = 0;
    const PctRec *rec = (const PctRec *)c->h_pct;
    if (n_samples) *n_samples = rec->n;
    if (a) *a = rec->a;
    if (b) *b = rec->b;
    if (gamma) *gamma = rec->gamma;
    if (thr) *thr = rec->thr;
    if (n_positive) *n_positive = (int64_t)(*(const unsigned long long *)((const char *)c->h_pct + 72));
    if (commit && rec->n > 0) mask_volume_fused_commit(c, c->tail_dst);
    return NL_OK;
}

extern "C" int nl_mask_volume_dev(nl_ctx *c, int64_t sz, int64_t sy, int64_t sx, double q, int64_t *n_samples, float *a, float *b, float *gamma,
                                  float *thr, char *err, size_t errlen) {
    NL_ENTER(c);
    int rc;
    if ((rc = pct_buffers(c, err, errlen))) return rc;
    Lattice L; FieldSrc fs;
    if ((rc = make_lattice(c, sz, sy, sx, L, err, errlen))) return rc;
    if ((rc = make_field(c, NL_FIELD_FRANGI, fs, err, errlen))) return rc;
    const i64 total = L.cz * L.cy * L.cx;
    if (total > c->n) return nl_fail(err, errlen, NL_EINVAL, "lattice larger than the volume");
    float *stage = nullptr;
    for (int k = 0; k < 3; ++k) if (k != c->i_gauss && c->f[k] != c->f[c->i_vmax]) stage = c->f[k];
    if (!stage) return nl_fail(err, errlen, NL_ESTATE, "no free volume for the samples");
    unsigned int *d_n = (unsigned int *)((char *)c->d_pct + 64);
    NL_HIP(zero_small(d_n, 4, c->stream));
    if (total > 0) {
        ProfScope ps(c, "sample");
        sample_gather_pos_kernel<<<(unsigned)((total + 255) / 256), 256, 0, c->stream>>>(fs, geom(c), L, stage, d_n);
        NL_CHECK_LAUNCH();
    }
    if ((rc = pct_enqueue(c, stage, d_n, total, (float)q, err, errlen))) return rc;
    int dst;
    if ((rc = mask_volume_enqueue(c, 0.0f, &((PctRec *)c->d_pct)->thr, &dst, err, errlen))) return rc;
    NL_HIP(hipMemcpyAsync(c->h_pct, c->d_pct, 64, hipMemcpyDeviceToHost, c->stream));
    NL_HIP(hipStreamSynchronize(c->stream));
    const PctRec *rec = (const PctRec *)c->h_pct;
    if (n_samples) *n_samples = rec->n;
    if (a) *a = rec->a;
    if (b) *b = rec->b;
    if (gamma) *gamma = rec->gamma;
    if (thr) *thr = rec->thr;
    if (rec->n > 0) mask_volume_commit(c, dst);
    return NL_OK;
}

extern "C" int nl_debug_percentile(nl_ctx *c, const float *values, int64_t n, double q, float *thr, float *a, float *b, char *err, size_t errlen) {
    NL_ENTER(c);
    if (!values || n < 1 || n > c->n) return nl_fail(err, errlen, NL_EINVAL, "bad sample array");
    int rc;
    if ((rc = pct_buffers(c, err, errlen))) return rc;
    float *stage = c->f[(c->i_gauss + 1) % 3];
    unsigned int *d_n = (unsigned int *)((char *)c->d_pct + 64);
    const unsigned int un = (unsigned int)n;
    NL_HIP(hipMemcpyAsync(stage, values, (size_t)n * 4, hipMemcpyHostToDevice, c->stream));
    NL_HIP(hipMemcpyAsync(d_n, &un, 4, hipMemcpyHostToDevice, c->stream));
    NL_HIP(hipStreamSynchronize(c->stream));
    const int keep = c->fuse_reduce; c->fuse_reduce = 0;
    rc = pct_enqueue(c, stage, d_n, n, (float)q, err, errlen);
    c->fuse_reduce = keep;
    if (rc) return rc;
    NL_HIP(hipMemcpyAsync(c->h_pct, c->d_pct, 64, hipMemcpyDeviceToHost, c->stream));
    NL_HIP(hipStreamSynchronize(c->stream));
    const PctRec *rec = (const PctRec *)c->h_pct;
    if (thr) *thr = rec->thr;
    if (a) *a = rec->a;
    if (b) *b = rec->b;
    return NL_OK;
}

int store_planes(nl_ctx *c, const void *dev_base, void *host, size_t elem, int64_t z0, int64_t z1, char *err, size_t errlen) {
    if (!host || z0 < 0 || z1 > c->nzl || z0 >= z1) return nl_fail(err, errlen, NL_EINVAL, "bad plane range [%lld,%lld)", (i64)z0, (i64)z1);
    const i64 plane = c->ny * c->nx;
    NL_HIP(hipMemcpyAsync(host, (const char *)dev_base + (size_t)z0 * plane * elem, (size_t)(z1 - z0) * plane * elem,
                          hipMemcpyDeviceToHost, c->stream));
    NL_HIP(hipStreamSynchronize(c->stream));
    return NL_OK;
}

extern "C" int nl_filter_store(nl_ctx *c, float *host, int64_t z0, int64_t z1, char *err, size_t errlen) {
    NL_ENTER(c);
    NL_KEEP_LABBITS(c);
    NL_KEEP_SUPPORT(c);
    return store_planes(c, c->f[c->i_vmax], host, 4, z0, z1, err, errlen);
}
extern "C" int nl_gauss_store(nl_ctx *c, float *host, int64_t z0, int64_t z1, char *err, size_t errlen) {
    NL_ENTER(c);
    return store_planes(c, gauss_cur(c), host, 4, z0, z1, err, errlen);
}

static float *field_ptr(nl_ctx *c, int field) {
    if (field == NL_FIELD_GAUSS) return gauss_cur(c);
    if (field == NL_FIELD_FRANGI) return c->f[c->i_vmax];
    return nullptr;
}

extern "C" int nl_planes_get(nl_ctx *c, int field, int64_t z0, int64_t z1, float *host, char *err, size_t errlen) {
    NL_ENTER(c);
    float *p = field_ptr(c, field);
    if (!p) return nl_fail(err, errlen, NL_EINVAL, "nl_planes_get: field %d has no volume", field);
    return store_planes(c, p, host, 4, z0, z1, err, errlen);
}

extern "C" int nl_planes_put(nl_ctx *c, int field, int64_t z0, int64_t z1, const float *host, char *err, size_t errlen) {
    NL_ENTER(c);
    float *p = field_ptr(c, field);
    c->fsq_cache_valid = 0;
    if (!p || !host || z0 < 0 || z1 > c->nzl || z0 >= z1) return nl_fail(err, errlen, NL_EINVAL, "nl_planes_put: bad field or plane range");
    const i64 plane = c->ny * c->nx;
    NL_HIP(hipMemcpyAsync(p + z0 * plane, host, (size_t)(z1 - z0) * plane * 4, hipMemcpyHostToDevice, c->stream));
    NL_HIP(hipStreamSynchronize(c->stream));
    return NL_OK;
}


extern "C" int nl_comm_unique_id(char *id128, char *err, size_t errlen) {
    if (!id128) return nl_fail(err, errlen, NL_EINVAL, "id buffer is NULL");
    ncclUniqueId id;
    {
        (void)hipGetLastError();
        ncclResult_t r_ = rccl().GetUniqueId(&id);
        if (r_ != ncclSuccess) return nl_fail(err, errlen, NL_ECOMM, "ncclGetUniqueId: %s", rccl().GetErrorString(r_));
    }
    static_assert(sizeof(id) == 128, "ncclUniqueId is 128 bytes");
    memcpy(id128, &id, 128);
    return NL_OK;
}

extern "C" int nl_comm_loopback_id(char *id128, char *err, size_t errlen) {
    if (!id128) return nl_fail(err, errlen, NL_EINVAL, "id buffer is NULL");
    lb::get_unique_id(id128);
    return NL_OK;
}

struct PooledComm { int device, world, rank, role; ncclComm_t comm; };
static std::mutex g_comm_pool_mu;
static std::vector<PooledComm> g_comm_pool;
static ncclComm_t comm_pool_take(int device, int world, int rank, int role) {
    std::lock_guard<std::mutex> lk(g_comm_pool_mu);
    for (size_t i = 0; i < g_comm_pool.size(); ++i) {
        const PooledComm &p = g_comm_pool[i];
        if (p.device == device && p.world == world && p.rank == rank && p.role == role) {
            ncclComm_t c = p.comm;
            g_comm_pool.erase(g_comm_pool.begin() + (long)i);
            return c;
        }
    }
    return nullptr;
}
static void comm_release(nl_ctx *c, void *comm, int role) {
    if (!comm) return;
    if (lb::is_ours(comm) || c->comm_poisoned || getenv("NELLIE_DESTROY_COMMS")) { rccl().CommDestroy((ncclComm_t)comm); return; }
    std::lock_guard<std::mutex> lk(g_comm_pool_mu);
    g_comm_pool.push_back(PooledComm{c->device, c->world, c->rank, role, (ncclComm_t)comm});
}
static int comm_acquire(nl_ctx *c, int world, int rank, const char *id128, int role, ncclComm_t *out, char *err, size_t errlen) {
    ncclUniqueId id;
    memcpy(&id, id128, 128);
    if (!lb::is_loopback_id(id128)) {
        ncclComm_t pooled = comm_pool_take(c->device, world, rank, role);
        if (pooled) { *out = pooled; return NL_OK; }
    }
    (void)hipGetLastError();
    NL_NCCL(rccl().CommInitRank(out, world, id, rank));
// ... 159 lines not shown
    const float *h = (const float *)c->h_ag;
    for (int r = 0; r < W; ++r) {
        unsigned int k; memcpy(&k, h + (size_t)r * blk, 4);
        if ((i64)k > block_items) return nl_fail(err, errlen, NL_ESTATE, "rank %d reports %u samples in a block of %lld", r, k, (long long)block_items);
        counts[r] = (int64_t)k;
        if (total + (i64)k > cap || (k && !out)) return nl_fail(err, errlen, NL_EINVAL, "output capacity %lld too small", (long long)cap);
        if (k) memcpy(out + total, h + (size_t)r * blk + 1, (size_t)k * 4);
        total += (i64)k;
    }
    return NL_OK;
}

extern "C" int nl_allgather_bytes(nl_ctx *c, const void *send, int64_t nbytes, void *recv, int64_t max_bytes, int64_t *bytes_of,
                                  char *err, size_t errlen) {
    NL_ENTER(c);
    NL_KEEP_SUPPORT(c);
    if (!c->comm) return nl_fail(err, errlen, NL_ESTATE, "nl_allgather_bytes before nl_comm_init");
    if (nbytes < 0 || max_bytes < 1 || nbytes > max_bytes || !recv || !bytes_of || (nbytes && !send))
        return nl_fail(err, errlen, NL_EINVAL, "bad all-gather arguments");
    const int W = c->world;
    long long *hs = (long long *)c->h_small;
    hs[0] = nbytes;
    NL_HIP(hipMemcpyAsync(c->d_small, hs, 8, hipMemcpyHostToDevice, c->stream));
    NL_NCCL(rccl().AllGather(c->d_small, (char *)c->d_small + 64, 1, ncclInt64, (ncclComm_t)c->comm, c->stream));
    NL_HIP(hipMemcpyAsync(hs, (char *)c->d_small + 64, (size_t)W * 8, hipMemcpyDeviceToHost, c->stream));
    NL_HIP(hipStreamSynchronize(c->stream));
    for (int r = 0; r < W; ++r) { bytes_of[r] = hs[r]; if (hs[r] > max_bytes) return nl_fail(err, errlen, NL_EINVAL, "rank %d sends %lld bytes, more than max_bytes = %lld", r, hs[r], (long long)max_bytes); }
    const size_t need = (size_t)max_bytes * (size_t)(W + 1);
    if (need > c->ag_cap) {
        if (c->d_ag) hipFree(c->d_ag);
        c->d_ag = nullptr; c->ag_cap = 0;
        NL_HIP(hipMalloc(&c->d_ag, need));
        c->ag_cap = need;
    }
    char *d_send = (char *)c->d_ag, *d_recv = d_send + max_bytes;
    if (nbytes) NL_HIP(hipMemcpyAsync(d_send, send, (size_t)nbytes, hipMemcpyHostToDevice, c->stream));
    NL_NCCL(rccl().AllGather(d_send, d_recv, (size_t)max_bytes, ncclChar, (ncclComm_t)c->comm, c->stream));
    NL_HIP(hipMemcpyAsync(recv, d_recv, (size_t)max_bytes * W, hipMemcpyDeviceToHost, c->stream));
    NL_HIP(hipStreamSynchronize(c->stream));
    return NL_OK;
}

extern "C" int nl_allgather_var(nl_ctx *c, const void *send, int64_t nbytes, void **recv, int64_t *stride, int64_t *bytes_of,
                                char *err, size_t errlen) {
    NL_ENTER(c);
    NL_KEEP_SUPPORT(c);
    if (!c->comm) return nl_fail(err, errlen, NL_ESTATE, "nl_allgather_var before nl_comm_init");
    if (nbytes < 0 || !recv || !stride || !bytes_of || (nbytes && !send)) return nl_fail(err, errlen, NL_EINVAL, "bad all-gather arguments");
    const int W = c->world;
    long long *hs = (long long *)c->h_small;
    hs[0] = nbytes;
    NL_HIP(hipMemcpyAsync(c->d_small, hs, 8, hipMemcpyHostToDevice, c->stream));
    NL_NCCL(rccl().AllGather(c->d_small, (char *)c->d_small + 64, 1, ncclInt64, (ncclComm_t)c->comm, c->stream));
    NL_HIP(hipMemcpyAsync(hs, (char *)c->d_small + 64, (size_t)W * 8, hipMemcpyDeviceToHost, c->stream));
    NL_HIP(hipStreamSynchronize(c->stream));
    long long mx = 16;
    for (int r = 0; r < W; ++r) { bytes_of[r] = hs[r]; if (hs[r] > mx) mx = hs[r]; }
    mx = (mx + 15) & ~15ll;
    const size_t need = (size_t)mx * (size_t)(W + 1);
    if (need > c->ag_cap) {
        if (c->d_ag) hipFree(c->d_ag);
        c->d_ag = nullptr; c->ag_cap = 0;
        NL_HIP(hipMalloc(&c->d_ag, need + need / 2));
        c->ag_cap = need + need / 2;
    }
    if ((size_t)mx * W > c->h_ag_cap) {
        if (c->h_ag) hipHostFree(c->h_ag);
        c->h_ag = nullptr; c->h_ag_cap = 0;
        const size_t cap = (size_t)mx * W * 3 / 2;
        NL_HIP(hipHostMalloc(&c->h_ag, cap, hipHostMallocDefault));
        c->h_ag_cap = cap;
    }
    char *d_send = (char *)c->d_ag, *d_recv = d_send + mx;
    if (nbytes) NL_HIP(hipMemcpyAsync(d_send, send, (size_t)nbytes, hipMemcpyHostToDevice, c->stream));
    NL_NCCL(rccl().AllGather(d_send, d_recv, (size_t)mx, ncclChar, (ncclComm_t)c->comm, c->stream));
    NL_HIP(hipMemcpyAsync(c->h_ag, d_recv, (size_t)mx * W, hipMemcpyDeviceToHost, c->stream));
    NL_HIP(hipStreamSynchronize(c->stream));
    *recv = c->h_ag; *stride = mx;
    return NL_OK;
}

extern "C" int nl_flat_sample_gather(nl_ctx *c, int field, int64_t offset, int64_t step, float *out, int64_t cap, int64_t *n,
                                     char *err, size_t errlen) {
    NL_ENTER(c);
    NL_KEEP_SUPPORT(c);
    if (step < 1 || offset < 0) return nl_fail(err, errlen, NL_EINVAL, "bad offset/step");
    if (field != NL_FIELD_FRANGI && field != NL_FIELD_GAUSS) return nl_fail(err, errlen, NL_EINVAL, "flat sampling supports GAUSS/FRANGI");
    const i64 plane = c->ny * c->nx;
    const i64 g_begin = (c->gz0 + c->own_lo) * plane, g_end = (c->gz0 + c->own_hi) * plane;
    i64 k0 = 0;
    if (g_begin > offset) k0 = (g_begin - offset + step - 1) / step;
    i64 k1 = (g_end > offset) ? (g_end - offset + step - 1) / step : 0;
    const i64 count = k1 > k0 ? k1 - k0 : 0;
    if (n) *n = count;
    if (count == 0 || (!out && cap == 0)) return NL_OK;
    if (!out || cap < count) return nl_fail(err, errlen, NL_EINVAL, "output capacity %lld < %lld samples", (i64)cap, count);
    const float *src = (field == NL_FIELD_FRANGI) ? c->f[c->i_vmax] : gauss_cur(c);
    float *stage = nullptr;
    for (int k = 0; k < 3; ++k) if (k != c->i_gauss && c->f[k] != src) { stage = c->f[k]; break; }
    {
        ProfScope ps(c, "sample");
        flat_gather_kernel<<<(unsigned)((count + 255) / 256), 256, 0, c->stream>>>(src, -c->gz0 * plane, offset + k0 * step, step, count, stage);
        NL_CHECK_LAUNCH();
    }
    NL_HIP(hipMemcpyAsync(out, stage, (size_t)count * 4, hipMemcpyDeviceToHost, c->stream));
    NL_HIP(hipStreamSynchronize(c->stream));
    return NL_OK;
}

extern "C" int nl_flat_sample_gather_positive(nl_ctx *c, int field, int64_t offset, int64_t step, float *out, int64_t cap,
                                              int64_t *n, char *err, size_t errlen) {
    NL_ENTER(c);
    NL_KEEP_SUPPORT(c);
    if (step < 1 || offset < 0) return nl_fail(err, errlen, NL_EINVAL, "bad offset/step");
    if (field != NL_FIELD_FRANGI && field != NL_FIELD_GAUSS) return nl_fail(err, errlen, NL_EINVAL, "flat sampling supports GAUSS/FRANGI");
    const i64 plane = c->ny * c->nx;
    const i64 g_begin = (c->gz0 + c->own_lo) * plane, g_end = (c->gz0 + c->own_hi) * plane;
    i64 k0 = 0;
    if (g_begin > offset) k0 = (g_begin - offset + step - 1) / step;
    i64 k1 = (g_end > offset) ? (g_end - offset + step - 1) / step : 0;
    const i64 count = k1 > k0 ? k1 - k0 : 0;
    if (n) *n = 0;
    if (count == 0) return NL_OK;
    if (!out || cap < count) return nl_fail(err, errlen, NL_EINVAL, "output capacity %lld < %lld samples", (i64)cap, count);
    const float *src = (field == NL_FIELD_FRANGI) ? c->f[c->i_vmax] : gauss_cur(c);
    float *stage = nullptr;
    for (int k = 0; k < 3; ++k) if (k != c->i_gauss && c->f[k] != src) { stage = c->f[k]; break; }
    unsigned int *d_n = (unsigned int *)c->d_small;
    NL_HIP(zero_small(d_n, 4, c->stream));
    {
        ProfScope ps(c, "sample");
        flat_gather_pos_kernel<<<(unsigned)((count + 255) / 256), 256, 0, c->stream>>>(src, -c->gz0 * plane, offset + k0 * step, step, count, stage, d_n);
        NL_CHECK_LAUNCH();
    }
    return fetch_counted(c, stage, d_n, count, out, cap, n, err, errlen);
}


extern "C" int nl_ctx_info(nl_ctx *c, const char *key, double *value) {
    if (!c || !key || !value) return NL_EINVAL;
    if (!strcmp(key, "fast_div")) *value = c->fast_div2 ? 2 : c->fast_div;
    else if (!strcmp(key, "hessian_tile_rows")) *value = hv_rs(c) ? 2 * hv_rs(c) : hm_ty();
    else if (!strcmp(key, "hv_variants")) *value = NL_HV_VARIANTS;
    else if (!strcmp(key, "vesselness_one_pass")) *value = c->spec_ok;
    else if (!strcmp(key, "chain_available")) *value = (c->two_d || (c->spec_ok && hv_rs(c))) ? 1 : 0;
    else if (!strcmp(key, "last_fsq_min")) *value = c->last_fsq_min;
    else if (!strcmp(key, "last_spec_overflow")) *value = c->last_spec_overflow;
    else if (!strcmp(key, "last_label_sparse")) *value = c->last_label_sparse;
    else if (!strcmp(key, "device_bytes")) *value = (double)nl_ctx_bytes(c->nzl, c->ny, c->nx);
    else if (!strcmp(key, "gauss_yx_max_r")) *value = getenv("NELLIE_NO_FUSED_YX") ? 0 : GM_MAX_R;
    else if (!strcmp(key, "queue_entries")) {
        if (hipSetDevice(c->device) != hipSuccess) return NL_EHIP;
        if (c->side_pending && hipStreamSynchronize(c->side) != hipSuccess) return NL_EHIP;
        const unsigned nreg = c->spec_nregions;
        std::vector<unsigned int> h(nreg);
        if (nreg && (hipMemcpyAsync(h.data(), c->d_vq_count, (size_t)nreg * 4, hipMemcpyDeviceToHost, c->stream) != hipSuccess ||
                     hipStreamSynchronize(c->stream) != hipSuccess)) return NL_EHIP;
        double t = 0.0;
        for (unsigned k = 0; k < nreg; ++k) t += (double)h[k];
        *value = t;
    }
    else if (!strcmp(key, "nan_hessian")) {
        if (hipSetDevice(c->device) != hipSuccess) return NL_EHIP;
        unsigned int flag = 0;
        if (c->side_pending && hipStreamSynchronize(c->side) != hipSuccess) return NL_EHIP;
        if (hipMemcpyAsync(&flag, (char *)c->d_small + NL_NAN_FLAG_OFF, 4, hipMemcpyDeviceToHost, c->stream) != hipSuccess ||
            hipStreamSynchronize(c->stream) != hipSuccess) return NL_EHIP;
        *value = flag ? 1.0 : 0.0;
    }
    else return NL_EINVAL;
    return NL_OK;
}

extern "C" int nl_debug_eig_frangi(nl_ctx *c, const float *h6, int64_t n, int impl, float alpha_sq, float beta_sq,
                                   float gamma_sq, float *out4, char *err, size_t errlen) {
    NL_ENTER(c);
    if (!h6 || !out4 || n < 1 || n * 6 > c->n) return nl_fail(err, errlen, NL_EINVAL, "bad debug batch (n=%lld)", (i64)n);
    float *d_in = c->f[(c->i_gauss + 1) % 3], *d_out = c->f[(c->i_gauss + 2) % 3];
    NL_HIP(hipMemcpyAsync(d_in, h6, (size_t)n * 24, hipMemcpyHostToDevice, c->stream));
    debug_eig_kernel<<<(unsigned)((n + 255) / 256), 256, 0, c->stream>>>(d_in, n, impl, alpha_sq, beta_sq, gamma_sq, d_out);
    NL_CHECK_LAUNCH();
    NL_HIP(hipMemcpyAsync(out4, d_out, (size_t)n * 16, hipMemcpyDeviceToHost, c->stream));
    NL_HIP(hipStreamSynchronize(c->stream));
    return NL_OK;
}

extern "C" int nl_timer_begin(nl_ctx *c, char *err, size_t errlen) {
    NL_ENTER(c);
    NL_HIP(hipEventRecord(c->t0, c->stream));
    return NL_OK;
}
extern "C" int nl_timer_end_ms(nl_ctx *c, float *ms, char *err, size_t errlen) {
    NL_ENTER(c);
    NL_HIP(hipEventRecord(c->t1, c->stream));
    NL_HIP(hipEventSynchronize(c->t1));
    float t = 0;
    NL_HIP(hipEventElapsedTime(&t, c->t0, c->t1));
    if (ms) *ms = t;
    return NL_OK;
}
extern "C" int nl_prof_enable(nl_ctx *c, int on) {
    if (!c) return NL_OK;
    if (on && !c->prof_on) {
        hipSetDevice(c->device);
        size_t used = 0;
        for (auto &kv : c->prof) used += kv.second.size();
        while (c->prof_pool.size() + used < 1024) {
            ProfRec r;
            if (hipEventCreate(&r.a) != hipSuccess) break;
            if (hipEventCreate(&r.b) != hipSuccess) { hipEventDestroy(r.a); break; }
            c->prof_pool.push_back(r);
        }
    }
    c->prof_on = on;
    return NL_OK;
}
extern "C" int nl_prof_reset(nl_ctx *c) {
    if (!c) return NL_OK;
    hipSetDevice(c->device);
    hipStreamSynchronize(c->stream);
    hipStreamSynchronize(c->side);
    for (auto &kv : c->prof) for (auto &r : kv.second) c->prof_pool.push_back(r);
    c->prof.clear();
    c->prof_sum.clear();
    return NL_OK;
}
extern "C" int nl_prof_get(nl_ctx *c, const char *name, double *ms, int64_t *launches) {
    if (!c || !name) return NL_EINVAL;
    hipSetDevice(c->device);
    hipStreamSynchronize(c->stream);
    hipStreamSynchronize(c->side);
// ... 10 lines not shown
```

nellie_amd/csrc/nellie_label.hip:

```cpp
#include "nl_host.h"
#include "label_voxels.inc"
#include "label_runs.inc"
#include "pack_out.inc"
#include "network.inc"

extern "C" int nl_label_load_frangi(nl_ctx *c, const float *host, int64_t z0, int64_t z1, char *err, size_t errlen) {
    NL_ENTER(c);
    if (!host || z0 < 0 || z1 > c->nzl || z0 >= z1) return nl_fail(err, errlen, NL_EINVAL, "bad plane range [%lld,%lld)", (i64)z0, (i64)z1);
    const i64 plane = c->ny * c->nx;
    c->i_vmax = 3; c->i_gauss = 0; c->i_labels = -1;
    NL_HIP(hipMemcpyAsync(c->f[c->i_vmax] + z0 * plane, host, (size_t)(z1 - z0) * plane * 4, hipMemcpyHostToDevice, c->stream));
    NL_HIP(hipStreamSynchronize(c->stream));
    c->frangi_ready = 1;
    return NL_OK;
}

extern "C" int nl_label_intensity_mask_planes(nl_ctx *c, const void *host_original, int dtype, double thresh, int64_t z0, int64_t z1,
                                              char *err, size_t errlen) {
    NL_ENTER(c);
    if (z0 < 0 || z1 > c->nzl || z0 >= z1) return nl_fail(err, errlen, NL_EINVAL, "bad plane range [%lld,%lld)", (i64)z0, (i64)z1);
    const i64 count = (z1 - z0) * c->ny * c->nx;
    const size_t es = dtype_size(dtype);
    if (!es || !host_original) return nl_fail(err, errlen, NL_EINVAL, "bad original image (dtype code %d)", dtype);
    void *raw = nullptr;
    NL_HIP(hipMalloc(&raw, (size_t)count * es));
    hipError_t e = hipMemcpyAsync(raw, host_original, (size_t)count * es, hipMemcpyHostToDevice, c->stream);
    if (e != hipSuccess) { hipFree(raw); return nl_fail(err, errlen, NL_EHIP, "upload of the original image failed: %s", hipGetErrorString(e)); }
    float *fr = c->f[c->i_vmax] + z0 * c->ny * c->nx;
    const unsigned int g = grid1d(count);
    switch (dtype) {
        case NL_U8: intensity_mask_kernel<uint8_t><<<g, 256, 0, c->stream>>>((const uint8_t *)raw, fr, thresh, count); break;
        case NL_I8: intensity_mask_kernel<int8_t><<<g, 256, 0, c->stream>>>((const int8_t *)raw, fr, thresh, count); break;
        case NL_U16: intensity_mask_kernel<uint16_t><<<g, 256, 0, c->stream>>>((const uint16_t *)raw, fr, thresh, count); break;
        case NL_I16: intensity_mask_kernel<int16_t><<<g, 256, 0, c->stream>>>((const int16_t *)raw, fr, thresh, count); break;
        case NL_U32: intensity_mask_kernel<uint32_t><<<g, 256, 0, c->stream>>>((const uint32_t *)raw, fr, thresh, count); break;
        case NL_I32: intensity_mask_kernel<int32_t><<<g, 256, 0, c->stream>>>((const int32_t *)raw, fr, thresh, count); break;
        case NL_F32: intensity_mask_kernel<float><<<g, 256, 0, c->stream>>>((const float *)raw, fr, thresh, count); break;
        case NL_F64: intensity_mask_kernel<double><<<g, 256, 0, c->stream>>>((const double *)raw, fr, thresh, count); break;
        case NL_U64: intensity_mask_kernel<uint64_t><<<g, 256, 0, c->stream>>>((const uint64_t *)raw, fr, thresh, count); break;
        case NL_I64: intensity_mask_kernel<int64_t><<<g, 256, 0, c->stream>>>((const int64_t *)raw, fr, thresh, count); break;
    }
    e = hipGetLastError();
    hipStreamSynchronize(c->stream);
    hipFree(raw);
    if (e != hipSuccess) return nl_fail(err, errlen, NL_EHIP, "intensity mask kernel: %s", hipGetErrorString(e));
    return NL_OK;
}
extern "C" int nl_label_intensity_mask(nl_ctx *c, const void *host_original, int dtype, double thresh, char *err, size_t errlen) {
    if (!c) return nl_fail(err, errlen, NL_EINVAL, "ctx is NULL");
    return nl_label_intensity_mask_planes(c, host_original, dtype, thresh, 0, c->nzl, err, errlen);
}

template <int FG, int CONN>
static int run_ccl(nl_ctx *c, const uint8_t *mask, int *L, char *err, size_t errlen) {
    const i64 nrows = c->nzl * c->ny;
    const i64 waves = nrows * ((c->nx + 63) / 64);
    ccl_init_kernel<FG><<<(unsigned)((waves * 64 + 255) / 256), 256, 0, c->stream>>>(mask, L, c->nx, nrows);
    NL_CHECK_LAUNCH();
    const dim3 grid((unsigned)((c->nx + 255) / 256), (unsigned)c->ny, (unsigned)c->nzl);
    ccl_merge_kernel<FG, CONN><<<grid, 256, 0, c->stream>>>(mask, L, c->nzl, c->ny, c->nx);
    NL_CHECK_LAUNCH();
    ccl_flatten_kernel<<<grid1d(c->n), 256, 0, c->stream>>>(L, c->n);
    NL_CHECK_LAUNCH();
    return NL_OK;
}

static int label_run_voxels(nl_ctx *c, int has_thr, float thr, int64_t min_area, int fill_holes, int64_t *n_labels,
                            char *err, size_t errlen) {
    int free_idx[3], nf = 0;
    for (int k = 0; k < 4; ++k) if (k != c->i_vmax) free_idx[nf++] = k;
    int *L = (int *)c->f[free_idx[0]];
    int *aux = (int *)c->f[free_idx[1]];
    int *out = (int *)c->f[free_idx[2]];
    uint8_t *mA = c->m[1], *mB = c->m[2], *flag = c->m[0];
    const i64 n = c->n;
    const i64 nrows = c->nzl * c->ny;
    const i64 waves = nrows * ((c->nx + 63) / 64);
    int rc;
    ProfScope ps(c, "label");
    threshold_kernel<<<grid1d(n), 256, 0, c->stream>>>(c->f[c->i_vmax], mA, has_thr, thr, n);
    NL_CHECK_LAUNCH();
    if (fill_holes) {
        if ((rc = run_ccl<0, 6>(c, mA, L, err, errlen))) return rc;
        clear_root_flags_kernel<<<grid1d(n), 256, 0, c->stream>>>(L, flag, n);
        NL_CHECK_LAUNCH();
        border_mark_kernel<<<grid1d(n), 256, 0, c->stream>>>(L, flag, geom(c));
        NL_CHECK_LAUNCH();
        fill_holes_apply_kernel<<<grid1d(n), 256, 0, c->stream>>>(L, flag, mA, n);
        NL_CHECK_LAUNCH();
    }
    if ((rc = run_ccl<1, 26>(c, mA, L, err, errlen))) return rc;
    zero_at_roots_kernel<<<grid1d(n), 256, 0, c->stream>>>(L, aux, n);
    NL_CHECK_LAUNCH();
    area_count_kernel<<<grid1d(waves * 64, 256, 256 * 16), 256, 0, c->stream>>>(L, aux, c->nx, nrows);
    NL_CHECK_LAUNCH();
    const int ma = (int)(min_area > 0x7fffffff ? 0x7fffffff : min_area);
    keep_large_kernel<<<grid1d(n), 256, 0, c->stream>>>(L, aux, mB, ma, n);
    NL_CHECK_LAUNCH();
    {
        const dim3 grid((unsigned)((c->nx + 255) / 256), (unsigned)c->ny, (unsigned)c->nzl);
        majority_kernel<<<grid, 256, 0, c->stream>>>(mB, mA, geom(c));
        NL_CHECK_LAUNCH();
    }
    if ((rc = run_ccl<1, 26>(c, mA, L, err, errlen))) return rc;
    const i64 nblk = (n + SCAN_CHUNK - 1) / SCAN_CHUNK;
    unsigned int *blk = (unsigned int *)c->d_blk;
    unsigned long long *d_total = (unsigned long long *)c->d_small;
    root_count_kernel<<<(unsigned)nblk, 256, 0, c->stream>>>(L, n, nullptr, n, blk);
    NL_CHECK_LAUNCH();
    blk_scan_kernel<<<1, 1024, 0, c->stream>>>(blk, nblk, d_total);
    NL_CHECK_LAUNCH();
    root_assign_kernel<<<(unsigned)nblk, 256, 0, c->stream>>>(L, n, nullptr, n, blk, aux);
    NL_CHECK_LAUNCH();
    relabel_kernel<<<grid1d(n), 256, 0, c->stream>>>(L, aux, out, n);
    NL_CHECK_LAUNCH();
    NL_HIP(hipMemcpyAsync(c->h_small, d_total, 8, hipMemcpyDeviceToHost, c->stream));
    NL_HIP(hipStreamSynchronize(c->stream));
    if (n_labels) *n_labels = (int64_t)(*(unsigned long long *)c->h_small);
    c->i_labels = free_idx[2];
    return NL_OK;
}


static int scan_excl_u32(nl_ctx *c, const unsigned int *in, unsigned int *out, i64 n, char *err, size_t errlen) {
    const i64 nblk = (n + SCAN_CHUNK - 1) / SCAN_CHUNK;
    unsigned int *blk = (unsigned int *)c->d_blk;
    unsigned long long *d_total = (unsigned long long *)c->d_small + 16;
    chunk_sum_kernel<<<(unsigned)nblk, 256, 0, c->stream>>>(in, n, blk);
    NL_CHECK_LAUNCH();
    blk_scan_kernel<<<1, 1024, 0, c->stream>>>(blk, nblk, d_total);
    NL_CHECK_LAUNCH();
    chunk_scan_kernel<<<(unsigned)nblk, 256, 0, c->stream>>>(in, out, n, blk);
    NL_CHECK_LAUNCH();
    return NL_OK;
}

struct RunSet { RunRec *runs; int *parent; unsigned int *row_off; i64 nruns; int *proot = nullptr; int *link = nullptr; bool proot_valid = false;
                bool host_count = true; i64 cap = 0;
                RunN rn() const { return RunN{host_count ? nullptr : n_ptr, nruns, cap}; }
                const unsigned int *n_ptr = nullptr; };
static unsigned run_blocks(const RunSet &rs, i64 nrows, int per_block = 256) {
    if (rs.host_count) return (unsigned)((rs.nruns + per_block - 1) / per_block > 0 ? (rs.nruns + per_block - 1) / per_block : 1);
    i64 b = nrows / 64;
    if (b < 256) b = 256;
    if (b > 8192) b = 8192;
    return (unsigned)b;
}

struct LabelGeo {
    i64 nz, ny, nx;
    i64 nrows; int wpr; i64 nwords;
    unsigned int *rows;
    unsigned long long *bitsA, *bitsB;
    i64 paint_row0, paint_row1;
    int *paint_out;
    int *link_scratch = nullptr;
    int zf_lo = 0, zf_hi = -2;
    i64 gz0 = 0, gnz = 0;
    bool rank_independent_bands = false;
    bool whole_frame_paint = false;
};
static void label_geo_whole(LabelGeo &g) { g.zf_lo = 0; g.zf_hi = (int)g.nz - 1; g.gz0 = 0; g.gnz = g.nz; }

template <int CONN>
static int build_components(nl_ctx *c, const LabelGeo &g, const unsigned long long *bits, int invert, RunSet &rs, i64 cap,
                            bool *overflow, char *err, size_t errlen) {
    unsigned int *counts = g.rows, *row_off = g.rows + (g.nrows + 2);
    NL_HIP(zero_small(counts + g.nrows, 4, c->stream));
    if (g.wpr <= 64) {
        int P = 1;
        while (P < g.wpr) P <<= 1;
        const i64 groups = (g.nrows + 64 / P - 1) / (64 / P);
        rl_count_wave_kernel<<<grid1d(groups * 64, 256, 16384), 256, 0, c->stream>>>(bits, invert, counts, g.nrows, g.wpr, (int)g.nx, P);
    }
    else rl_count_kernel<<<(unsigned)((g.nrows + 255) / 256), 256, 0, c->stream>>>(bits, invert, counts, g.nrows, g.wpr, (int)g.nx);
    NL_CHECK_LAUNCH();
    int rc = scan_excl_u32(c, counts, row_off, g.nrows + 1, err, errlen);
    if (rc) return rc;
    rs.row_off = row_off; rs.n_ptr = row_off + g.nrows; rs.cap = cap;
    rs.proot_valid = false;
    *overflow = false;
    unsigned int *d_ovf = (unsigned int *)c->d_small + 60;
    if (rs.host_count) {
        NL_HIP(hipMemcpyAsync(c->h_small, row_off + g.nrows, 4, hipMemcpyDeviceToHost, c->stream));
        NL_HIP(hipStreamSynchronize(c->stream));
        rs.nruns = (i64)(*(unsigned int *)c->h_small);
        *overflow = rs.nruns > cap;
        if (*overflow || rs.nruns == 0) return NL_OK;
    } else {
        rs.nruns = -1;
    }
    static int two_level = -1;
    if (two_level < 0) { const char *e = getenv("NELLIE_UF_PLANES"); two_level = (e && !atoi(e)) ? 0 : 1; }
    static int seg_target = -1;
    if (seg_target < 0) { const char *e = getenv("NELLIE_UF_SEG_WGS"); seg_target = (e && atoi(e) > 0) ? atoi(e) : 1024; }
    int seg_shift = 5;
    if (g.rank_independent_bands) {
        const i64 want = seg_target == 1 ? 1 : 8;
        while (((g.ny + ((i64)1 << seg_shift) - 1) >> seg_shift) > want) ++seg_shift;
    } else {
        const i64 want = (seg_target + g.nz - 1) / g.nz;
        while (((g.ny + ((i64)1 << seg_shift) - 1) >> seg_shift) > want) ++seg_shift;
    }
    const int nseg = (int)((g.ny + ((i64)1 << seg_shift) - 1) >> seg_shift);
    const size_t seg_bytes = (size_t)g.nz * nseg;
    if (two_level && rs.proot && rs.link && seg_bytes > c->seg_done_cap) {
        if (c->d_seg_done) { NL_HIP(hipStreamSynchronize(c->stream)); NL_HIP(hipFree(c->d_seg_done)); c->d_seg_done = nullptr; c->seg_done_cap = 0; }
        const size_t want_bytes = seg_bytes < 8192 ? 8192 : seg_bytes;
        NL_HIP(hipMalloc((void **)&c->d_seg_done, want_bytes));
        c->seg_done_cap = want_bytes;
    }
    const bool lvl2 = two_level && rs.proot && rs.link;
    int *link = lvl2 ? rs.link : nullptr;
    if (g.wpr <= 30)
        rl_emit_kernel<true><<<(unsigned)((g.nrows + 255) / 256), 256, (size_t)256 * (g.wpr + 1) * 8, c->stream>>>(bits, invert, row_off, rs.runs, rs.parent, g.nrows, g.wpr, (int)g.nx, link, cap, d_ovf);
    else
        rl_emit_kernel<false><<<(unsigned)((g.nrows + 255) / 256), 256, 0, c->stream>>>(bits, invert, row_off, rs.runs, rs.parent, g.nrows, g.wpr, (int)g.nx, link, cap, d_ovf);
    NL_CHECK_LAUNCH();
    const unsigned gr = run_blocks(rs, g.nrows);
    const RunN rn = rs.rn();
    if (lvl2) {
        uint8_t *seg_done = c->d_seg_done;
        rl_union_plane_kernel<CONN><<<(unsigned)(g.nz * nseg), 256, 0, c->stream>>>(rs.runs, row_off, rs.parent, rs.proot, (int)g.ny,
                                                                         CONN == 6 ? 1 : 0, g.zf_lo, g.zf_hi, (int)g.nx, seg_done, seg_shift, nseg, rn);
        rl_union_cross_kernel<CONN><<<gr, 256, 0, c->stream>>>(rs.runs, row_off, rs.parent, rs.proot, rs.link, rn, (int)g.ny,
                                                               CONN == 6 ? 1 : 0, g.zf_lo, g.zf_hi, (int)g.nx, seg_done, seg_shift, nseg);
        rs.proot_valid = true;
    } else {
        rl_union_kernel<CONN><<<gr, 256, 0, c->stream>>>(rs.runs, row_off, rs.parent, rn, (int)g.ny,
                                                         CONN == 6 ? 1 : 0, g.zf_lo, g.zf_hi, (int)g.nx);
    }
    NL_CHECK_LAUNCH();
    ccl_flatten_kernel<<<gr, 256, 0, c->stream>>>(rs.parent, rs.nruns, rn.p, cap);
    NL_CHECK_LAUNCH();
    return NL_OK;
}

static int pack_enqueue_fwd(nl_ctx *c, int with_labels, const float *frangi, const int *labels, char *err, size_t errlen);
static int number_and_paint(nl_ctx *c, const LabelGeo &g, const RunSet &rs, int *aux, int64_t *n_labels, char *err, size_t errlen,
                            bool *overflow = nullptr) {
    unsigned long long total = 0;
    unsigned int *blk = (unsigned int *)c->d_blk;
    unsigned long long *d_total = (unsigned long long *)c->d_small;
    const bool any = !rs.host_count || rs.nruns > 0;
    if (any) {
        const RunN rn = rs.rn();
        const unsigned nb = rs.host_count ? (unsigned)((rs.nruns + SCAN_CHUNK - 1) / SCAN_CHUNK) : run_blocks(rs, g.nrows / 16 + 1);
        root_count_kernel<<<nb, 256, 0, c->stream>>>(rs.parent, rs.nruns, rn.p, rs.cap, blk);
        NL_CHECK_LAUNCH();
        blk_scan_kernel<<<1, 1024, 0, c->stream>>>(blk, rs.host_count ? (rs.nruns + SCAN_CHUNK - 1) / SCAN_CHUNK : 0, d_total, rn.p, rs.cap);
        NL_CHECK_LAUNCH();
        root_assign_kernel<<<nb, 256, 0, c->stream>>>(rs.parent, rs.nruns, rn.p, rs.cap, blk, aux);
        NL_CHECK_LAUNCH();
        NL_HIP(hipMemcpyAsync(c->h_small, d_total, 8, hipMemcpyDeviceToHost, c->stream));
        NL_HIP(hipMemcpyAsync((char *)c->h_small + 8, (unsigned int *)c->d_small + 60, 4, hipMemcpyDeviceToHost, c->stream));
    }
    rl_paint_kernel<<<grid1d((g.paint_row1 - g.paint_row0) * 64, 256, (i64)1 << 22), 256, 0, c->stream>>>(
        g.bitsA, rs.row_off, rs.parent, aux, g.paint_out, g.paint_row0, g.paint_row1, g.wpr, (int)g.nx);
    NL_CHECK_LAUNCH();
    bool packed = false;
    if (c->pack_with_label && g.whole_frame_paint && c->own_lo == 0 && c->own_hi == c->nzl && c->frangi_ready) {
        const int rcp = pack_enqueue_fwd(c, 1, c->f[c->i_vmax], g.paint_out, err, errlen);
        if (rcp) return rcp;
        packed = true;
    }
    NL_HIP(hipStreamSynchronize(c->stream));
    if (any) total = *(unsigned long long *)c->h_small;
    if (overflow) *overflow = any && !rs.host_count && *(unsigned int *)((char *)c->h_small + 8) != 0;
    c->pack_pending = (packed && !(overflow && *overflow)) ? 1 : 0;
    if (n_labels) *n_labels = (int64_t)total;
    return NL_OK;
}

static int label_core(nl_ctx *c, const LabelGeo &g, int64_t min_area, int fill_holes, int64_t *n_labels, bool *overflow,
                      char *err, size_t errlen) {
    int free_idx[3], nf = 0;
    for (int k = 0; k < 4; ++k) if (k != c->i_vmax) free_idx[nf++] = k;
    const i64 cap = c->n / 2;
    RunSet rs;
    rs.runs = (RunRec *)c->f[free_idx[0]];
    rs.parent = (int *)c->f[free_idx[1]];
    int *aux = rs.parent + cap;
    rs.proot = aux;
    rs.link = g.link_scratch;
    uint8_t *flag = c->m[0];
    const VolGeom vg{g.nz, g.ny, g.nx, g.gz0, g.gnz};
    int rc;
    *overflow = false;
    static int dev_count = -1;
    if (dev_count < 0) { const char *e = getenv("NELLIE_LABEL_HOST_COUNTS"); dev_count = (e && atoi(e)) ? 0 : 1; }
    rs.host_count = !dev_count;
    NL_HIP(zero_small((unsigned int *)c->d_small + 60, 4, c->stream));
    auto known_empty = [&]() { return rs.host_count && rs.nruns == 0; };
    if (fill_holes) {
        if ((rc = build_components<6>(c, g, g.bitsA, 1, rs, cap, overflow, err, errlen))) return rc;
        if (*overflow) return NL_OK;
        if (!known_empty()) {
            const unsigned gr = run_blocks(rs, g.nrows);
            rl_fill_u8_kernel<<<gr, 256, 0, c->stream>>>(flag, rs.rn());
            rl_border_kernel<<<gr, 256, 0, c->stream>>>(rs.runs, rs.parent, flag, rs.rn(), vg);
            NL_CHECK_LAUNCH();
            rl_fill_kernel<<<gr, 256, 0, c->stream>>>(rs.runs, rs.parent, flag, g.bitsA, rs.rn(), g.wpr);
            NL_CHECK_LAUNCH();
        }
    }
    if ((rc = build_components<26>(c, g, g.bitsA, 0, rs, cap, overflow, err, errlen))) return rc;
    if (*overflow) return NL_OK;
    NL_HIP(hipMemsetAsync(g.bitsB, 0, (size_t)g.nwords * 8, c->stream));
    if (!known_empty()) {
        const unsigned gr = run_blocks(rs, g.nrows);
        rl_fill_u32_kernel<<<gr, 256, 0, c->stream>>>((unsigned int *)aux, 0u, rs.rn());
        rl_area_kernel<<<run_blocks(rs, g.nrows / 16 + 1, RL_CHUNK), 256, 0, c->stream>>>(rs.runs, rs.parent, aux, rs.rn());
        NL_CHECK_LAUNCH();
        const int ma = (int)(min_area > 0x7fffffff ? 0x7fffffff : min_area);
        rl_keep_kernel<<<gr, 256, 0, c->stream>>>(rs.runs, rs.parent, aux, ma, g.bitsB, rs.rn(), g.wpr);
        NL_CHECK_LAUNCH();
    }
    majority_bits_kernel<<<(unsigned)((g.nwords + 255) / 256), 256, 0, c->stream>>>(g.bitsB, g.bitsA, vg, g.wpr, 0, g.nz);
    NL_CHECK_LAUNCH();
    if ((rc = build_components<26>(c, g, g.bitsA, 0, rs, cap, overflow, err, errlen))) return rc;
    if (*overflow) return NL_OK;
    if ((rc = number_and_paint(c, g, rs, aux, n_labels, err, errlen, overflow))) return rc;
    if (*overflow) return NL_OK;
    c->i_labels = free_idx[2];
    return NL_OK;
}

static int label_out_index(const nl_ctx *c) {
    int last = -1;
    for (int k = 0; k < 4; ++k) if (k != c->i_vmax) last = k;
    return last;
}

extern "C" int nl_label_run(nl_ctx *c, int has_thr, float thr, int64_t min_area, int fill_holes, int64_t *n_labels,
                            char *err, size_t errlen) {
    NL_ENTER(c);
    if (!c->frangi_ready) return nl_fail(err, errlen, NL_ESTATE, "nl_label_run before a Frangi volume exists");
    if (c->nzl != c->gnz) return nl_fail(err, errlen, NL_EINVAL, "nl_label_run works on a whole volume (Z-slabs: nl_label_pack / nl_label_run_global)");
    static int force_voxel = -1;
    if (force_voxel < 0) { const char *e = getenv("NELLIE_LABEL_VOXEL"); force_voxel = (e && atoi(e)) ? 1 : 0; }
    if (force_voxel || c->nx > 65535) return label_run_voxels(c, has_thr, thr, min_area, fill_holes, n_labels, err, errlen);
    LabelGeo g;
    g.nz = c->nzl; g.ny = c->ny; g.nx = c->nx;
    g.nrows = c->nzl * c->ny; g.wpr = (int)((c->nx + 63) / 64); g.nwords = g.nrows * g.wpr;
    g.rows = c->d_rows;
    g.bitsA = (unsigned long long *)c->m[1]; g.bitsB = (unsigned long long *)c->m[2];
    g.paint_row0 = 0; g.paint_row1 = g.nrows; g.paint_out = (int *)c->f[label_out_index(c)];
    g.link_scratch = g.paint_out;
    label_geo_whole(g);
    g.whole_frame_paint = true;
    c->pack_pending = 0;
    ProfScope ps(c, "label");
    const unsigned long long *support = (c->support_epoch + 1 == c->epoch.load() && c->d_support && has_thr && thr >= 0.0f) ? c->d_support : nullptr;
    c->last_label_sparse = support ? 1 : 0;
    rl_threshold_pack_kernel<<<grid1d(g.nrows * 64, 256, support ? (i64)256 * 64 : (i64)1 << 22), 256, 0, c->stream>>>(c->f[c->i_vmax], support, g.bitsA, has_thr, thr,
                                                                                          (int)c->nx, g.nrows, g.wpr);
    NL_CHECK_LAUNCH();
    bool overflow = false;
    int rc = label_core(c, g, min_area, fill_holes, n_labels, &overflow, err, errlen);
    if (rc) return rc;
    if (overflow) return label_run_voxels(c, has_thr, thr, min_area, fill_holes, n_labels, err, errlen);
    c->labbits_epoch = c->epoch.load();
    return NL_OK;
}

static int ensure_global_label_buffers(nl_ctx *c, char *err, size_t errlen) {
    const i64 grows = c->gnz * c->ny;
    const int wpr = (int)((c->nx + 63) / 64);
    if (!c->gbits[0]) {
        NL_HIP(hipMalloc((void **)&c->gbits[0], (size_t)grows * wpr * 8));
        NL_HIP(hipMalloc((void **)&c->gbits[1], (size_t)grows * wpr * 8));
        NL_HIP(hipMalloc((void **)&c->grows, ((size_t)grows + 2) * 2 * 4));
        if ((grows + 1 + SCAN_CHUNK - 1) / SCAN_CHUNK + 1 > c->blk_cap) {
            hipFree(c->d_blk);
            c->blk_cap = (grows + 1 + SCAN_CHUNK - 1) / SCAN_CHUNK + 1;
            NL_HIP(hipMalloc(&c->d_blk, (size_t)c->blk_cap * 4));
        }
    }
    return NL_OK;
}

extern "C" int nl_label_pack(nl_ctx *c, int has_thr, float thr, char *err, size_t errlen) {
    NL_ENTER(c);
    if (!c->frangi_ready) return nl_fail(err, errlen, NL_ESTATE, "nl_label_pack before a Frangi volume exists");
    if (c->nx > 65535) return nl_fail(err, errlen, NL_EINVAL, "rows longer than 65535 voxels are not supported on Z-slabs");
    int rc = ensure_global_label_buffers(c, err, errlen);
    if (rc) return rc;
    const int wpr = (int)((c->nx + 63) / 64);
    const i64 own_rows = (c->own_hi - c->own_lo) * c->ny;
    const i64 row0 = (c->gz0 + c->own_lo) * c->ny;
    ProfScope ps(c, "label");
    rl_threshold_pack_kernel<<<grid1d(own_rows * 64, 256, (i64)1 << 22), 256, 0, c->stream>>>(
        c->f[c->i_vmax] + c->own_lo * c->ny * c->nx, nullptr, c->gbits[0] + row0 * wpr, has_thr, thr, (int)c->nx, own_rows, wpr);
    NL_CHECK_LAUNCH();
    return NL_OK;
}

extern "C" int nl_label_bits_get(nl_ctx *c, int64_t row0, int64_t nrows, uint64_t *host, char *err, size_t errlen) {
    NL_ENTER(c);
    const int wpr = (int)((c->nx + 63) / 64);
    if (!c->gbits[0] || !host || row0 < 0 || nrows < 1 || row0 + nrows > c->gnz * c->ny) return nl_fail(err, errlen, NL_EINVAL, "bad bit-mask row range");
    NL_HIP(hipMemcpyAsync(host, c->gbits[0] + row0 * wpr, (size_t)nrows * wpr * 8, hipMemcpyDeviceToHost, c->stream));
    NL_HIP(hipStreamSynchronize(c->stream));
    return NL_OK;
}
extern "C" int nl_label_bits_put(nl_ctx *c, int64_t row0, int64_t nrows, const uint64_t *host, char *err, size_t errlen) {
    NL_ENTER(c);
    const int wpr = (int)((c->nx + 63) / 64);
    if (!c->gbits[0] || !host || row0 < 0 || nrows < 1 || row0 + nrows > c->gnz * c->ny) return nl_fail(err, errlen, NL_EINVAL, "bad bit-mask row range");
    NL_HIP(hipMemcpyAsync(c->gbits[0] + row0 * wpr, host, (size_t)nrows * wpr * 8, hipMemcpyHostToDevice, c->stream));
    NL_HIP(hipStreamSynchronize(c->stream));
    return NL_OK;
}

extern "C" int nl_label_bits_allgather(nl_ctx *c, const int64_t *slab_plane0, char *err, size_t errlen) {
    NL_ENTER(c);
    if (!c->comm) return nl_fail(err, errlen, NL_ESTATE, "nl_label_bits_allgather before nl_comm_init");
    if (!c->gbits[0] || !slab_plane0) return nl_fail(err, errlen, NL_ESTATE, "nl_label_bits_allgather before nl_label_pack");
    const int wpr = (int)((c->nx + 63) / 64);
    ProfScope ps(c, "halo");
    NL_NCCL(rccl().GroupStart());
    for (int r = 0; r < c->world; ++r) {
        const i64 p0 = slab_plane0[r], p1 = slab_plane0[r + 1];
        unsigned long long *ptr = c->gbits[0] + p0 * c->ny * wpr;
        NL_NCCL(rccl().Broadcast(ptr, ptr, (size_t)((p1 - p0) * c->ny * wpr), ncclUint64, r, (ncclComm_t)c->comm, c->stream));
    }
    NL_NCCL(rccl().GroupEnd());
    return NL_OK;
}

extern "C" int nl_label_run_global(nl_ctx *c, int64_t min_area, int fill_holes, int64_t *n_labels, char *err, size_t errlen) {
    NL_ENTER(c);
    if (!c->gbits[0]) return nl_fail(err, errlen, NL_ESTATE, "nl_label_run_global before nl_label_pack");
    LabelGeo g;
    g.nz = c->gnz; g.ny = c->ny; g.nx = c->nx;
    g.nrows = c->gnz * c->ny; g.wpr = (int)((c->nx + 63) / 64); g.nwords = g.nrows * g.wpr;
    g.rows = c->grows;
    g.bitsA = c->gbits[0]; g.bitsB = c->gbits[1];
    g.paint_row0 = (c->gz0 + c->own_lo) * c->ny; g.paint_row1 = (c->gz0 + c->own_hi) * c->ny;
    g.paint_out = (int *)c->f[label_out_index(c)] + c->own_lo * c->ny * c->nx;
    label_geo_whole(g);
    ProfScope ps(c, "label");
    bool overflow = false;
    int rc = label_core(c, g, min_area, fill_holes, n_labels, &overflow, err, errlen);
// ... 217 lines not shown
    const unsigned gr = (unsigned)((rs.nruns + 255) / 256);
    if (c->sl_phase == SL_FILL) {
        if (rs.nruns) sl_fill_kernel<<<gr, 256, 0, c->stream>>>(rs.runs, rs.parent, c->m[0], g.bitsA, rs.nruns, g.wpr, sg.row_lo, sg.row_hi);
    } else {
        NL_HIP(hipMemsetAsync(g.bitsB + (i64)sg.row_lo * g.wpr, 0, (size_t)(sg.row_hi - sg.row_lo) * g.wpr * 8, c->stream));
        const int ma = (int)(min_area > 0x7fffffff ? 0x7fffffff : min_area);
        if (rs.nruns) sl_keep_kernel<<<gr, 256, 0, c->stream>>>(rs.runs, rs.parent, sg.aux, ma, g.bitsB, rs.nruns, g.wpr, sg.row_lo, sg.row_hi);
    }
    NL_CHECK_LAUNCH();
    return NL_OK;
}

extern "C" int nl_slab_majority(nl_ctx *c, char *err, size_t errlen) {
    NL_ENTER(c);
    SlabGeo sg; int rc = slab_geo(c, sg, err, errlen); if (rc) return rc;
    LabelGeo &g = sg.g;
    ProfScope ps(c, "label");
    const i64 z_lo = c->own_lo - c->sl_e0, z_hi = c->own_hi - c->sl_e0;
    majority_bits_kernel<<<(unsigned)(((z_hi - z_lo) * g.ny * g.wpr + 255) / 256), 256, 0, c->stream>>>(g.bitsB, g.bitsA, VolGeom{g.nz, g.ny, g.nx, g.gz0, g.gnz}, g.wpr, z_lo, z_hi);
    NL_CHECK_LAUNCH();
    return NL_OK;
}

extern "C" int nl_slab_number(nl_ctx *c, int64_t n_clear, const int32_t *clear, int64_t n_set, const int32_t *set, int64_t *n_local,
                              int32_t *ids_of_set, char *err, size_t errlen) {
    NL_ENTER(c);
    if (c->sl_phase != SL_NUMBER) return nl_fail(err, errlen, NL_ESTATE, "nl_slab_number outside the numbering phase");
    if (n_clear < 0 || n_set < 0 || (n_clear && !clear) || (n_set && (!set || !ids_of_set)) || n_clear + n_set > c->n / 4) return nl_fail(err, errlen, NL_EINVAL, "bad selection lists");
    SlabGeo sg; int rc = slab_geo(c, sg, err, errlen); if (rc) return rc;
    RunSet &rs = sg.rs;
    ProfScope ps(c, "label");
    unsigned long long total = 0;
    if (rs.nruns) {
        sl_select_kernel<<<(unsigned)((rs.nruns + 255) / 256), 256, 0, c->stream>>>(rs.runs, rs.parent, sg.sel, rs.nruns, sg.row_lo, sg.row_hi);
        int *d_idx = (int *)(sg.scan + rs.nruns);
        if (rs.nruns + n_clear + 2 * n_set > sg.cap) return nl_fail(err, errlen, NL_ENOMEM, "selection lists do not fit the scratch volume [out of memory]");
        if ((rc = slab_host_stage(c, (size_t)(n_clear + n_set) + 2 + (size_t)n_set, err, errlen))) return rc;
        if (n_clear) memcpy(c->h_sl, clear, (size_t)n_clear * 4);
        if (n_set) memcpy(c->h_sl + n_clear, set, (size_t)n_set * 4);
        if (n_clear + n_set) NL_HIP(hipMemcpyAsync(d_idx, c->h_sl, (size_t)(n_clear + n_set) * 4, hipMemcpyHostToDevice, c->stream));
        if (n_clear) sl_set_u32_kernel<<<(unsigned)((n_clear + 255) / 256), 256, 0, c->stream>>>(sg.sel, d_idx, (int)n_clear, 0u);
        if (n_set) sl_set_u32_kernel<<<(unsigned)((n_set + 255) / 256), 256, 0, c->stream>>>(sg.sel, d_idx + n_clear, (int)n_set, 1u);
        NL_CHECK_LAUNCH();
        if ((rc = scan_excl_u32(c, sg.sel, sg.scan, rs.nruns, err, errlen))) return rc;
        int *h_back = c->h_sl + n_clear + n_set;
        int *d_out = d_idx + n_clear + n_set;
        if (n_set) {
            sl_gather_kernel<<<(unsigned)((n_set + 255) / 256), 256, 0, c->stream>>>(sg.scan, d_idx + n_clear, d_out, (int)n_set, 1);
            NL_CHECK_LAUNCH();
            NL_HIP(hipMemcpyAsync(h_back + 2, d_out, (size_t)n_set * 4, hipMemcpyDeviceToHost, c->stream));
        }
        NL_HIP(hipMemcpyAsync(h_back, sg.scan + rs.nruns - 1, 4, hipMemcpyDeviceToHost, c->stream));
        NL_HIP(hipMemcpyAsync(h_back + 1, sg.sel + rs.nruns - 1, 4, hipMemcpyDeviceToHost, c->stream));
        NL_HIP(hipStreamSynchronize(c->stream));
        total = (unsigned long long)(unsigned int)h_back[0] + (unsigned int)h_back[1];
        if (n_set) memcpy(ids_of_set, h_back + 2, (size_t)n_set * 4);
    } else if (n_set) {
        return nl_fail(err, errlen, NL_EINVAL, "selection on an empty run set");
    }
    if (n_local) *n_local = (int64_t)total;
    c->sl_numbered = 1;
    return NL_OK;
}

extern "C" int nl_slab_paint(nl_ctx *c, int64_t base, int64_t n, const int32_t *roots, const int32_t *labels, char *err, size_t errlen) {
    NL_ENTER(c);
    if (!c->sl_numbered) return nl_fail(err, errlen, NL_ESTATE, "nl_slab_paint before nl_slab_number");
    if (n < 0 || (n && (!roots || !labels))) return nl_fail(err, errlen, NL_EINVAL, "bad label patch");
    SlabGeo sg; int rc = slab_geo(c, sg, err, errlen); if (rc) return rc;
    LabelGeo &g = sg.g; RunSet &rs = sg.rs;
    ProfScope ps(c, "label");
    if (rs.nruns) {
        sl_ids_kernel<<<(unsigned)((rs.nruns + 255) / 256), 256, 0, c->stream>>>(sg.sel, sg.scan, (int)base, sg.aux, rs.nruns);
        if (n) {
            if (rs.nruns + 2 * n > sg.cap) return nl_fail(err, errlen, NL_ENOMEM, "label patch does not fit the scratch volume [out of memory]");
            int *d_idx = (int *)(sg.scan + rs.nruns), *d_val = d_idx + n;
            if ((rc = slab_host_stage(c, (size_t)2 * n, err, errlen))) return rc;
            memcpy(c->h_sl, roots, (size_t)n * 4); memcpy(c->h_sl + n, labels, (size_t)n * 4);
            NL_HIP(hipMemcpyAsync(d_idx, c->h_sl, (size_t)2 * n * 4, hipMemcpyHostToDevice, c->stream));
            sl_patch_kernel<<<(unsigned)((n + 255) / 256), 256, 0, c->stream>>>(sg.aux, nullptr, d_idx, d_val, (int)n);
        }
        NL_CHECK_LAUNCH();
    }
    rl_paint_kernel<<<grid1d((g.paint_row1 - g.paint_row0) * 64, 256, (i64)1 << 22), 256, 0, c->stream>>>(
        g.bitsA, rs.row_off, rs.parent, sg.aux, g.paint_out, g.paint_row0, g.paint_row1, g.wpr, (int)g.nx);
    NL_CHECK_LAUNCH();
    NL_HIP(hipStreamSynchronize(c->stream));
    c->i_labels = sg.out_idx;
    c->sl_numbered = 0; c->sl_phase = -1;
    return NL_OK;
}

extern "C" int nl_host_slab_join(int world, const int32_t *blobs, int64_t block_ints, int64_t cap, int64_t *n_nodes, int64_t *n_comp,
                                 int64_t *node_rank, int32_t *node_root, int64_t *node_val, int64_t *node_comp, char *err, size_t errlen) {
    if (world < 1 || !blobs || block_ints < 8 || !n_nodes || !n_comp) return nl_fail(err, errlen, NL_EINVAL, "bad join arguments");
    struct Tab { const int32_t *root[4], *val[4]; int n[4]; };
    std::vector<Tab> tabs((size_t)world);
    std::vector<std::vector<int32_t>> uniq((size_t)world);
    std::vector<i64> base((size_t)world + 1, 0);
    for (int r = 0; r < world; ++r) {
        const int32_t *b = blobs + (size_t)r * (size_t)block_ints;
        i64 total = 0;
        for (int k = 0; k < 4; ++k) { if (b[k] < 0) return nl_fail(err, errlen, NL_EINVAL, "negative table size"); total += b[k]; }
        if (8 + 2 * total > block_ints) return nl_fail(err, errlen, NL_EINVAL, "rank %d: table of %lld entries exceeds the block", r, (long long)total);
        i64 off = 8;
        for (int k = 0; k < 4; ++k) { tabs[r].n[k] = b[k]; tabs[r].root[k] = b + off; tabs[r].val[k] = b + total + off; off += b[k]; }
        auto &u = uniq[r];
        u.assign(b + 8, b + 8 + total);
        std::sort(u.begin(), u.end());
        u.erase(std::unique(u.begin(), u.end()), u.end());
        base[r + 1] = base[r] + (i64)u.size();
    }
    const i64 n = base[world];
    *n_nodes = n;
    if (n > cap) { *n_comp = 0; return nl_fail(err, errlen, NL_EINVAL, "the output arrays hold %lld nodes, the tables name %lld (n_nodes says how many to allocate)", (long long)cap, (long long)n); }
    auto node_of = [&](int r, int32_t root) -> i64 {
        const auto &u = uniq[r];
        return base[r] + (i64)(std::lower_bound(u.begin(), u.end(), root) - u.begin());
    };
    std::vector<i64> par((size_t)n);
    for (i64 i = 0; i < n; ++i) par[i] = i;
    auto find = [&](i64 i) -> i64 { while (par[i] != i) { par[i] = par[par[i]]; i = par[i]; } return i; };
    std::vector<char> have((size_t)n, 0);
    for (int r = 0; r < world; ++r)
        for (int k = 0; k < 4; ++k)
            for (int e = 0; e < tabs[r].n[k]; ++e) {
                const i64 v = node_of(r, tabs[r].root[k][e]);
                if (!have[v]) { have[v] = 1; node_rank[v] = r; node_root[v] = tabs[r].root[k][e]; node_val[v] = tabs[r].val[k][e]; }
            }
    for (int r = 0; r + 1 < world; ++r)
        for (int pair = 0; pair < 2; ++pair) {
            const int mine = 2 + pair, theirs = pair;
            if (tabs[r].n[mine] != tabs[r + 1].n[theirs])
                return nl_fail(err, errlen, NL_EINVAL, "slab tables of ranks %d and %d disagree (%d vs %d entries): the ghost bit planes are stale",
                               r, r + 1, tabs[r].n[mine], tabs[r + 1].n[theirs]);
            for (int e = 0; e < tabs[r].n[mine]; ++e) {
                i64 a = find(node_of(r, tabs[r].root[mine][e])), b = find(node_of(r + 1, tabs[r + 1].root[theirs][e]));
                if (a != b) { if (a < b) par[b] = a; else par[a] = b; }
            }
        }
    i64 nc = 0;
    std::vector<i64> id((size_t)n, -1);
    for (i64 i = 0; i < n; ++i) { const i64 rt = find(i); if (id[rt] < 0) id[rt] = nc++; node_comp[i] = id[rt]; }
    *n_comp = nc;
    return NL_OK;
}

extern "C" int nl_label_store(nl_ctx *c, int32_t *host, int64_t z0, int64_t z1, char *err, size_t errlen) {
    NL_ENTER(c);
    NL_KEEP_LABBITS(c);
    if (c->i_labels < 0) return nl_fail(err, errlen, NL_ESTATE, "nl_label_store before nl_label_run");
    return store_planes(c, c->f[c->i_labels], host, 4, z0, z1, err, errlen);
}

extern "C" int nl_skel_pixel_class(nl_ctx *c, const int32_t *skel_host, uint8_t *pixel_class_host, int64_t *n_skel,
                                   char *err, size_t errlen) {
    NL_ENTER(c);
    NL_JOIN_SIDE(c);
    if (!skel_host) return nl_fail(err, errlen, NL_EINVAL, "nl_skel_pixel_class: skel is NULL");
    if (c->own_lo != 0 || c->own_hi != c->nzl || c->gnz != c->nzl) return nl_fail(err, errlen, NL_EINVAL, "the Network kernels run on a whole volume");
    const int wpr = (int)((c->nx + 63) / 64);
    const i64 nrows = c->nzl * c->ny, nw = nrows * wpr;
    ProfScope ps(c, "network");
    NL_HIP(hipMemcpyAsync(c->f[3], skel_host, (size_t)c->n * 4, hipMemcpyHostToDevice, c->stream));
    unsigned long long *skel = (unsigned long long *)c->m[1], *branch = (unsigned long long *)c->m[2];
    nl_launch_pack_labels(grid1d(nw * 64, 256, (i64)1 << 20), c->stream, (const int *)c->f[3], skel, (int)c->nx, nrows, wpr);
    NL_CHECK_LAUNCH();
// ... 355 lines not shown
```

nellie_amd/csrc/nl_common.h:

```cpp
#pragma once
#include <atomic>
#include <hip/hip_runtime.h>
#include <stdarg.h>
#include <stdint.h>
#include <stdio.h>
#include <string.h>
#include <string>
#include <vector>
#include <map>

#include "../../include/nellie_amd.h"

typedef long long i64;

struct ProfRec { hipEvent_t a, b; };

struct nl_ctx {
    int device = 0;
    hipStream_t stream = nullptr;
    i64 nzl = 0, ny = 0, nx = 0;
    i64 gz0 = 0, gnz = 0;
    i64 own_lo = 0, own_hi = 0;
    i64 n = 0;

    float *f[4] = {nullptr, nullptr, nullptr, nullptr};
    uint8_t *m[3] = {nullptr, nullptr, nullptr};
    int i_gauss = 0;
    int i_vmax = 3;
    int i_labels = -1;

    void *d_input = nullptr;
    int input_dtype = -1;
    int input_borrowed = 0;
    hipStream_t copy_in = nullptr, copy_out = nullptr;
    void *d_in_slot[2] = {nullptr, nullptr};
    size_t in_bytes[2] = {0, 0};
    int in_dtype[2] = {-1, -1};
    hipEvent_t ev_in[2] = {nullptr, nullptr};
    hipEvent_t ev_staged = nullptr, ev_fetched = nullptr;
    float *d_stage_fr = nullptr;
    void *d_pack = nullptr; size_t pack_cap = 0;
    int pack_with_label = 0;
    int pack_pending = 0;
    int *d_stage_lab = nullptr;
    void *d_small = nullptr;
    void *h_small = nullptr;
    void *h_prefix = nullptr;
    float *d_vq = nullptr;
    unsigned int *d_vq_count = nullptr;
    int nw_state = 0;
    const float *mk_int = nullptr;
    float *mk_use = nullptr;
    float *mk_scratch = nullptr;
    std::atomic<unsigned long long> epoch{0};
    unsigned long long support_epoch = ~0ull - 8;
    const unsigned long long *d_support = nullptr;
    unsigned long long labbits_epoch = ~0ull - 8;
    int last_label_sparse = 0;
    unsigned char *mk_act = nullptr; size_t mk_act_cap = 0;
    int mk_act_valid = 0;
    int mk_ntiles = 0;
    int mk_state = 0;
    int mk_first_scale = 1;
    int two_d = 0;
    float *d_2d[4] = {nullptr, nullptr, nullptr, nullptr};
    float *d_fsq_cache = nullptr;
    i64 fsq_cache_cap = 0, fsq_cache_key[3] = {0, 0, 0};
    int fsq_cache_valid = 0;
    float *gauss_ext = nullptr;
    int vq_chunks = 1;
    int spec_ok = 0;
    int spec_valid = 0;
    float spec_lo = 0, spec_hi = 0;
    i64 spec_z0 = 0, spec_z1 = 0;
    unsigned int spec_nregions = 0;
    int spec_qcap = 0;
    unsigned long long spec_count = 0;
    hipStream_t side = nullptr;
    hipEvent_t ev_side = nullptr, ev_main = nullptr;
    hipEvent_t ev_ahead = nullptr;
    int ahead_pending = 0, ahead_gauss = 0;
    int side_pending = 0;
    int def_resolve = 0;
    alignas(8) unsigned char def_vp[160] = {};
    unsigned long long *def_cnt = nullptr;
    const float *def_params = nullptr;
    int last_spec_overflow = 0;
    float last_fsq_min = 0;
    void *d_blk = nullptr;
    unsigned int *d_rows = nullptr;
    unsigned long long *gbits[2] = {nullptr, nullptr};
    unsigned int *grows = nullptr;
    int comm_poisoned = 0;
    i64 blk_cap = 0;
    i64 sl_e0 = 0, sl_e1 = 0;
    i64 sl_nruns = 0;
    int sl_phase = -1;
    int *d_sl = nullptr; size_t d_sl_ints = 0;
    int *h_sl = nullptr; size_t h_sl_ints = 0;
    int sl_capE = 0;
    int sl_numbered = 0;
    uint8_t *d_seg_done = nullptr; size_t seg_done_cap = 0;

    float hz = 1, hy = 1, hx = 1;
    float hz2 = 2, hy2 = 2, hx2 = 2;
    int have_spacing = 0;
    int fast_div = 0;
    int fast_div2 = 0;
    double chk_spacing[3] = {0, 0, 0};
    float frob_max_abs = 1.0f, frob_max_finite = 0.0f;
    int frangi_ready = 0;
    i64 vmax_zero_lo = 0, vmax_zero_hi = 0;
    int mask_slots_used = 0;
    hipEvent_t ev_chain = nullptr; int chain_copy_pending = 0;
    i64 gp_total = -1; float *gp_stage = nullptr;
    void *d_pct = nullptr;
    void *h_pct = nullptr;
    int tail_pending = 0, tail_dst = -1;
    void *d_chain = nullptr, *h_chain = nullptr;
    int chain_n = 0, chain_k = 0;
    double chain_par[16][3] = {};

    void *comm = nullptr;
    int fuse_reduce = 0;
    void *d_ag = nullptr; size_t ag_cap = 0;
    void *h_ag = nullptr; size_t h_ag_cap = 0;
    void *comm2 = nullptr;
    hipStream_t xstream = nullptr;
    hipEvent_t ev_x_main = nullptr, ev_x_done = nullptr;
    int halo_pending = 0;
    int world = 1, rank = 0;

    hipEvent_t t0 = nullptr, t1 = nullptr;
    int prof_on = 0;
    std::map<std::string, std::vector<ProfRec>> prof;
    std::map<std::string, std::pair<double, int64_t>> prof_sum;
    std::vector<ProfRec> prof_pool;
    std::vector<hipEvent_t> ev_pool;
};

static inline int nl_fail(char *err, size_t errlen, int code, const char *fmt, ...) {
// ... 55 lines not shown
```

nellie_amd/csrc/nl_host.h:

```cpp
#pragma once
#include <stdarg.h>
#include <stdlib.h>
#include <type_traits>
#include <thread>
#include <mutex>
#include <vector>
#include <dlfcn.h>
#include <rccl/rccl.h>
#include "nl_common.h"

#define NL_MASK_SLOTS 2
#define NL_VERSION "nellie_amd-hip 0.1.0 (gfx950)"
#define SCAN_CHUNK 4096

struct CommApi {
    std::atomic<int> n_real{0};
    ncclResult_t GetUniqueId(ncclUniqueId *id);
    ncclResult_t CommInitRank(ncclComm_t *comm, int world, ncclUniqueId id, int rank);
    ncclResult_t CommDestroy(ncclComm_t comm);
    const char *GetErrorString(ncclResult_t r);
    ncclResult_t GroupStart();
    ncclResult_t GroupEnd();
    ncclResult_t Send(const void *buf, size_t count, ncclDataType_t dt, int peer, ncclComm_t comm, hipStream_t st);
    ncclResult_t Recv(void *buf, size_t count, ncclDataType_t dt, int peer, ncclComm_t comm, hipStream_t st);
    ncclResult_t AllReduce(const void *src, void *dst, size_t count, ncclDataType_t dt, ncclRedOp_t op, ncclComm_t comm, hipStream_t st);
    ncclResult_t AllGather(const void *src, void *dst, size_t count, ncclDataType_t dt, ncclComm_t comm, hipStream_t st);
    ncclResult_t Broadcast(const void *src, void *dst, size_t count, ncclDataType_t dt, int root, ncclComm_t comm, hipStream_t st);
};
CommApi &rccl();

#include "device_math.inc"
#include "convert.inc"
#include "gauss_launch.h"

static inline dim3 grid2d_rows(i64 nx, i64 ny) {
    const i64 gx = (nx + 255) / 256;
    i64 gy = (1024 + gx - 1) / gx;
    if (gy > ny) gy = ny;
    if (gy < 1) gy = 1;
    return dim3((unsigned)gx, (unsigned)gy, 1);
}
static inline unsigned int grid1d(i64 n, int block = 256, i64 cap = 256 * 32) {
    i64 g = (n + block - 1) / block;
    if (g > cap) g = cap;
    if (g < 1) g = 1;
    return (unsigned int)g;
}

static __global__ void zero_words_kernel(unsigned int *p, int n) {
    for (int i = threadIdx.x; i < n; i += blockDim.x) p[i] = 0u;
}
static inline hipError_t zero_small(void *p, size_t bytes, hipStream_t st) {
    zero_words_kernel<<<1, 256, 0, st>>>((unsigned int *)p, (int)(bytes / 4));
    return hipGetLastError();
}

static float *gauss_cur(const nl_ctx *c) { return c->gauss_ext ? c->gauss_ext : c->f[c->i_gauss]; }
static VolGeom geom(const nl_ctx *c) {
    VolGeom v{c->nzl, c->ny, c->nx, c->gz0, c->gnz};
    static int forced = -1;
    if (forced < 0) { const char *e = getenv("NELLIE_GM_CHUNK"); forced = e ? atoi(e) : 0; }
    v.chunk = forced > 0 ? forced : (c->two_d ? 32 : (c->n >= ((i64)1 << 29) ? 256 : 128));
    return v;
}

static size_t dtype_size(int dt) {
    switch (dt) {
        case NL_U8: case NL_I8: return 1;
        case NL_U16: case NL_I16: return 2;
        case NL_U32: case NL_I32: case NL_F32: return 4;
        case NL_F64: case NL_U64: case NL_I64: return 8;
    }
    return 0;
}

#define NL_ENTER(c)                                                    \
    if (!(c)) return nl_fail(err, errlen, NL_EINVAL, "ctx is NULL");   \
    ++(c)->epoch;                                                      \
    NL_HIP(hipSetDevice((c)->device));

#define NL_ENTER_IO(c)                                                 \
    if (!(c)) return nl_fail(err, errlen, NL_EINVAL, "ctx is NULL");   \
    NL_HIP(hipSetDevice((c)->device));

#define NL_KEEP_SUPPORT(c) if ((c)->support_epoch + 1 == (c)->epoch.load()) (c)->support_epoch = (c)->epoch.load();
#define NL_KEEP_LABBITS(c) if ((c)->labbits_epoch + 1 == (c)->epoch.load()) (c)->labbits_epoch = (c)->epoch.load();

#define NL_JOIN_SIDE(c)                                                            \
    if ((c)->side_pending) {                                                       \
        NL_HIP(hipStreamWaitEvent((c)->stream, (c)->ev_side, 0));                  \
        (c)->side_pending = 0;                                                     \
    }

#define NL_NCCL(expr)                                                                                  \
    do {                                                                                               \
        ncclResult_t r_ = (expr);                                                                      \
        if (r_ != ncclSuccess) { c->comm_poisoned = 1; return nl_fail(err, errlen, NL_ECOMM, "%s: %s", #expr, rccl().GetErrorString(r_)); } \
    } while (0)


static inline bool fused(const nl_ctx *c) { return c->comm && c->fuse_reduce; }

int upload_convert(nl_ctx *c, const void *host, int dtype, float *dst, i64 count, char *err, size_t errlen);
int fetch_counted(nl_ctx *c, const float *stage, const unsigned int *d_n, i64 max_count, float *out, i64 cap, int64_t *n, char *err, size_t errlen);
int store_planes(nl_ctx *c, const void *dev_base, void *host, size_t elem, int64_t z0, int64_t z1, char *err, size_t errlen);
int64_t vq_alloc_entries(int64_t nzl, int64_t ny, int64_t nx);
bool gyx_tiled();
void nl_launch_threshold_pack(unsigned int grid, hipStream_t st, const float *f, const unsigned long long *support, unsigned long long *bits,
                              int has_thr, float thr, int nx, i64 nrows, int wpr, const float *thr_dev);
void nl_launch_pack_labels(unsigned int grid, hipStream_t st, const int *lab, unsigned long long *bits, int nx, i64 nrows, int wpr);
```

Baseline: 28290 Mvoxel/s.

## Pre-zero label output during the last Gaussian pass and skip zero fills in paint

On the final scale's fused Gaussian pass, the third volume buffer is zeroed as a side effect, and its pre-zeroed status is tracked with an epoch-guarded pointer across API calls. Label then paints into that buffer with a sparse paint kernel that skips empty rows and writes only set voxels. This removes a full-volume zero-write pass from the labeling hot path. In exchange, buffer-selection logic in the sampling and mask code must avoid or invalidate the pre-zeroed buffer, and the label link scratch needs re-zeroing, which adds stateful complexity.

```diff
diff --git a/nellie_amd/csrc/label_runs.inc b/nellie_amd/csrc/label_runs.inc
--- a/nellie_amd/csrc/label_runs.inc
+++ b/nellie_amd/csrc/label_runs.inc
@@ -539,6 +539,7 @@
     out[t] = res;
 }
 
+template <bool SPARSE>
 __global__ void __launch_bounds__(256)
 rl_paint_kernel(const unsigned long long *__restrict__ bits, const unsigned int *__restrict__ row_off, const int *__restrict__ parent,
                 const int *__restrict__ newid, int *__restrict__ out, i64 row0, i64 row1, int wpr, int nx) {
@@ -549,14 +550,17 @@
         unsigned int seen = seen0;
         int *orow = out + (row - row0) * nx;
         const bool vec = ((nx & 3) == 0) && ((reinterpret_cast<size_t>(orow) & 15) == 0);
+        if (SPARSE && nr == 0u) continue;
         if (nr == 0u && vec) {
             for (int q = lane; q < nx / 4; q += 64) reinterpret_cast<int4 *>(orow)[q] = make_int4(0, 0, 0, 0);
             continue;
         }
         const int lab_mine = ((unsigned int)lane < nr) ? newid[parent[seen0 + lane]] : 0;
         if (vec) {
+            if (!SPARSE) {
             for (int q = lane; q < nx / 4; q += 64) reinterpret_cast<int4 *>(orow)[q] = make_int4(0, 0, 0, 0);
             asm volatile("s_waitcnt vmcnt(0)" ::: "memory");
+            }
             unsigned long long carry = 0;
             int prev_w = -2;
             for (int wb = 0; wb < wpr; wb += 64) {
@@ -597,7 +601,7 @@
                 const unsigned int rl = set ? (seen - seen0) + (unsigned int)__builtin_popcountll(below) - 1u : 0u;
                 int lab = __shfl(lab_mine, (int)(rl & 63u), 64);
                 if (set && rl >= 64u) lab = newid[parent[seen0 + rl]];
-                if (x < nx) orow[x] = set ? lab : 0;
+                if (x < nx && (set || !SPARSE)) orow[x] = set ? lab : 0;
                 seen += (unsigned int)__builtin_popcountll(starts);
                 carry = v >> 63;
             }
diff --git a/nellie_amd/csrc/nellie_hip.hip b/nellie_amd/csrc/nellie_hip.hip
--- a/nellie_amd/csrc/nellie_hip.hip
+++ b/nellie_amd/csrc/nellie_hip.hip
@@ -433,6 +433,7 @@
     NL_JOIN_SIDE(c);
     if (!host || z0 < 0 || z1 > c->nzl || z0 >= z1) return nl_fail(err, errlen, NL_EINVAL, "bad plane range [%lld,%lld)", (i64)z0, (i64)z1);
     c->i_gauss = 0; c->i_vmax = 3; c->i_labels = -1; c->frangi_ready = 0;
+    c->pz_on = 0; c->prezero_used = 0;
     c->gauss_ext = nullptr;
     if (c->ahead_pending) NL_HIP(hipStreamWaitEvent(c->stream, c->ev_ahead, 0));
     c->ahead_pending = 0;
@@ -467,6 +468,7 @@
     NL_JOIN_SIDE(c);
     if (!c->d_input) return nl_fail(err, errlen, NL_ESTATE, "nl_filter_begin before nl_input_load");
     c->i_gauss = 0; c->i_vmax = 3; c->i_labels = -1; c->frangi_ready = 0;
+    c->pz_on = 0; c->prezero_used = 0;
     c->mask_slots_used = 0;
     c->gauss_ext = nullptr;
     if (c->ahead_pending) NL_HIP(hipStreamWaitEvent(c->stream, c->ev_ahead, 0));
@@ -538,9 +540,13 @@
         static int zero_in_passing = -1;
         if (zero_in_passing < 0) { const char *e = getenv("NELLIE_ZERO_IN_GAUSS"); zero_in_passing = (e && !atoi(e)) ? 0 : 1; }
         const bool zero = zero_in_passing && c->mask_slots_used == 0 && c->vmax_zero_hi == 0 && c->stream != c->side;
-        (void)gl_zyx(c, rz, ry, srcp, c->f[dst], v, z0, z1, gauss_ws_of(gw), gauss_ws_of(gy), zero ? c->f[c->i_vmax] : nullptr);
+        const bool ahead = c->stream == c->side;
+        const bool prezero = !zero && c->pz_on && c->chain_n > 0 && c->chain_k == c->chain_n - (ahead ? 2 : 1) && z0 == 0 && z1 == c->nzl;
+        float *third = c->f[(src + 2) % 3];
+        (void)gl_zyx(c, rz, ry, srcp, c->f[dst], v, z0, z1, gauss_ws_of(gw), gauss_ws_of(gy), zero ? c->f[c->i_vmax] : (prezero ? third : nullptr));
         if (zero) { c->vmax_zero_lo = z0; c->vmax_zero_hi = z1; }
         NL_CHECK_LAUNCH();
+        if (prezero) pz_set(c, third);
         src = dst; srcp = c->f[dst];
         fused_yx = true;
         wz = nullptr;
@@ -614,7 +620,7 @@
 }
 
 extern "C" int nl_gauss_commit(nl_ctx *c, char *err, size_t errlen) {
-    NL_ENTER(c);
+    NL_ENTER_KEEP_PZ(c);
     if (!c->ahead_pending) return nl_fail(err, errlen, NL_ESTATE, "nl_gauss_commit without nl_gauss_step_ahead");
     NL_HIP(hipStreamWaitEvent(c->stream, c->ev_ahead, 0));
     c->i_gauss = c->ahead_gauss;
@@ -1412,12 +1418,14 @@
     NL_CHECK_LAUNCH();
     c->chain_n = n_scales; c->chain_k = 0; c->chain_copy_pending = 0;
     c->def_resolve = 0;
+    const char *e_pz = getenv("NELLIE_PREZERO");
+    c->pz_on = (e_pz ? atoi(e_pz) != 0 : NL_PREZERO_DEFAULT) && !c->two_d && !c->comm && c->own_lo == 0 && c->own_hi == c->nzl && c->nzl == c->gnz;
     return NL_OK;
 }
 
 extern "C" int nl_chain_scale(nl_ctx *c, const double spacing[3], int64_t sz, int64_t sy, int64_t sx, double alpha_sq, double beta_sq,
                               double division, double margin, double test_scale, int64_t z0, int64_t z1, char *err, size_t errlen) {
-    NL_ENTER(c);
+    NL_ENTER_KEEP_PZ(c);
     if (!c->d_chain || c->chain_k >= c->chain_n) return nl_fail(err, errlen, NL_ESTATE, "nl_chain_scale outside nl_chain_begin .. nl_chain_finish");
     if (!(division != 0.0)) return nl_fail(err, errlen, NL_EINVAL, "the chain needs a non-zero threshold division");
     int rc;
@@ -1518,7 +1526,7 @@
 }
 
 extern "C" int nl_chain_flush(nl_ctx *c, char *err, size_t errlen) {
-    NL_ENTER(c);
+    NL_ENTER_KEEP_PZ(c);
     if (!c->d_chain || c->chain_k < 1) return nl_fail(err, errlen, NL_ESTATE, "nl_chain_flush without scales");
     { int rcd = resolve_deferred_launch(c, false, err, errlen); if (rcd) return rcd; }
     NL_JOIN_SIDE(c);
@@ -1529,7 +1537,7 @@
 }
 
 extern "C" int nl_chain_finish(nl_ctx *c, int *flags, double *gamma, double *max_abs, double *thr, int64_t *mask_count, char *err, size_t errlen) {
-    NL_ENTER(c);
+    NL_ENTER_KEEP_PZ(c);
     if (!c->d_chain || c->chain_k < 1) return nl_fail(err, errlen, NL_ESTATE, "nl_chain_finish without scales");
     const int n = c->chain_k;
     if (!c->chain_copy_pending) { int rcd = resolve_deferred_launch(c, false, err, errlen); if (rcd) return rcd; }
@@ -1550,7 +1558,7 @@
         if (thr) thr[k] = (double)h[k].thr;
         if (mask_count) mask_count[k] = (int64_t)(h[k].cnt_walk + h[k].cnt_resolve);
     }
-    c->chain_n = 0;
+    c->chain_n = 0; c->pz_on = 0;
     return NL_OK;
 }
 
@@ -1793,7 +1801,9 @@
 
 static int mask_volume_fused_enqueue(nl_ctx *c, float thr, const float *thr_dev, unsigned long long *d_cnt, int *dst_out, char *err, size_t errlen) {
     int dst = -1;
-    for (int k = 0; k < 3; ++k) if (k != c->i_gauss) { dst = k; break; }
+    for (int k = 0; k < 3; ++k) if (k != c->i_gauss && !pz_is(c, c->f[k])) { dst = k; break; }
+    if (dst < 0) for (int k = 0; k < 3; ++k) if (k != c->i_gauss) { dst = k; break; }
+    pz_touch(c, c->f[dst]);
     *dst_out = dst;
     NL_HIP(zero_small(d_cnt, 8, c->stream));
     ProfScope ps(c, "mask_volume");
@@ -1829,7 +1839,7 @@
 }
 
 extern "C" int nl_mask_volume_fused(nl_ctx *c, float thr, int64_t *n_positive, char *err, size_t errlen) {
-    NL_ENTER(c);
+    NL_ENTER_KEEP_PZ(c);
     if (c->mask_slots_used == 0) return nl_fail(err, errlen, NL_ESTATE, "nl_mask_volume_fused before any scale was evaluated");
     NL_JOIN_SIDE(c);
     unsigned long long *d_cnt = (unsigned long long *)c->d_small;
@@ -1870,7 +1880,7 @@
 }
 
 extern "C" int nl_tail_enqueue(nl_ctx *c, int64_t sz, int64_t sy, int64_t sx, double q, char *err, size_t errlen) {
-    NL_ENTER(c);
+    NL_ENTER_KEEP_PZ(c);
     if (c->mask_slots_used == 0) return nl_fail(err, errlen, NL_ESTATE, "nl_tail_enqueue before any scale was evaluated");
     if (c->two_d) return nl_fail(err, errlen, NL_EINVAL, "nl_tail_enqueue is the 3-D epilogue");
     int rc;
@@ -1882,6 +1892,7 @@
     if (total > c->n) return nl_fail(err, errlen, NL_EINVAL, "lattice larger than the volume");
     float *stage = c->f[(c->i_gauss + 1) % 3];
     if (stage == c->f[c->i_vmax]) return nl_fail(err, errlen, NL_ESTATE, "no free volume for the samples");
+    const bool stage_pz = pz_is(c, stage);
     unsigned int *d_n = (unsigned int *)((char *)c->d_pct + 64);
     unsigned long long *d_cnt = (unsigned long long *)((char *)c->d_pct + 72);
     NL_HIP(zero_small(d_n, 4, c->stream));
@@ -1891,6 +1902,7 @@
         NL_CHECK_LAUNCH();
     }
     if ((rc = pct_enqueue(c, stage, d_n, total, (float)q, err, errlen))) return rc;
+    if (stage_pz && total > 0) NL_HIP(hipMemsetAsync(stage, 0, (size_t)total * 4, c->stream));
     int dst;
     if ((rc = mask_volume_fused_enqueue(c, 0.0f, &((PctRec *)c->d_pct)->thr, d_cnt, &dst, err, errlen))) return rc;
     NL_HIP(hipMemcpyAsync(c->h_pct, c->d_pct, 80, hipMemcpyDeviceToHost, c->stream));
@@ -1900,7 +1912,7 @@
 
 extern "C" int nl_tail_finish(nl_ctx *c, int commit, int64_t *n_samples, float *a, float *b, float *gamma, float *thr, int64_t *n_positive,
                               char *err, size_t errlen) {
-    NL_ENTER(c);
+    NL_ENTER_KEEP_PZ(c);
     if (!c->tail_pending) return nl_fail(err, errlen, NL_ESTATE, "nl_tail_finish without nl_tail_enqueue");
     NL_HIP(hipStreamSynchronize(c->stream));
     c->tail_pending = 0;
@@ -1984,7 +1996,7 @@
 }
 
 extern "C" int nl_filter_store(nl_ctx *c, float *host, int64_t z0, int64_t z1, char *err, size_t errlen) {
-    NL_ENTER(c);
+    NL_ENTER_KEEP_PZ(c);
     NL_KEEP_LABBITS(c);
     NL_KEEP_SUPPORT(c);
     return store_planes(c, c->f[c->i_vmax], host, 4, z0, z1, err, errlen);
@@ -2310,7 +2322,7 @@
 
 extern "C" int nl_flat_sample_gather(nl_ctx *c, int field, int64_t offset, int64_t step, float *out, int64_t cap, int64_t *n,
                                      char *err, size_t errlen) {
-    NL_ENTER(c);
+    NL_ENTER_KEEP_PZ(c);
     NL_KEEP_SUPPORT(c);
     if (step < 1 || offset < 0) return nl_fail(err, errlen, NL_EINVAL, "bad offset/step");
     if (field != NL_FIELD_FRANGI && field != NL_FIELD_GAUSS) return nl_fail(err, errlen, NL_EINVAL, "flat sampling supports GAUSS/FRANGI");
@@ -2325,7 +2337,9 @@
     if (!out || cap < count) return nl_fail(err, errlen, NL_EINVAL, "output capacity %lld < %lld samples", (i64)cap, count);
     const float *src = (field == NL_FIELD_FRANGI) ? c->f[c->i_vmax] : gauss_cur(c);
     float *stage = nullptr;
-    for (int k = 0; k < 3; ++k) if (k != c->i_gauss && c->f[k] != src) { stage = c->f[k]; break; }
+    for (int k = 0; k < 3; ++k) if (k != c->i_gauss && c->f[k] != src && !pz_is(c, c->f[k])) { stage = c->f[k]; break; }
+    if (!stage) for (int k = 0; k < 3; ++k) if (k != c->i_gauss && c->f[k] != src) { stage = c->f[k]; break; }
+    pz_touch(c, stage);
     {
         ProfScope ps(c, "sample");
         flat_gather_kernel<<<(unsigned)((count + 255) / 256), 256, 0, c->stream>>>(src, -c->gz0 * plane, offset + k0 * step, step, count, stage);
@@ -2338,7 +2352,7 @@
 
 extern "C" int nl_flat_sample_gather_positive(nl_ctx *c, int field, int64_t offset, int64_t step, float *out, int64_t cap,
                                               int64_t *n, char *err, size_t errlen) {
-    NL_ENTER(c);
+    NL_ENTER_KEEP_PZ(c);
     NL_KEEP_SUPPORT(c);
     if (step < 1 || offset < 0) return nl_fail(err, errlen, NL_EINVAL, "bad offset/step");
     if (field != NL_FIELD_FRANGI && field != NL_FIELD_GAUSS) return nl_fail(err, errlen, NL_EINVAL, "flat sampling supports GAUSS/FRANGI");
@@ -2353,7 +2367,9 @@
     if (!out || cap < count) return nl_fail(err, errlen, NL_EINVAL, "output capacity %lld < %lld samples", (i64)cap, count);
     const float *src = (field == NL_FIELD_FRANGI) ? c->f[c->i_vmax] : gauss_cur(c);
     float *stage = nullptr;
-    for (int k = 0; k < 3; ++k) if (k != c->i_gauss && c->f[k] != src) { stage = c->f[k]; break; }
+    for (int k = 0; k < 3; ++k) if (k != c->i_gauss && c->f[k] != src && !pz_is(c, c->f[k])) { stage = c->f[k]; break; }
+    if (!stage) for (int k = 0; k < 3; ++k) if (k != c->i_gauss && c->f[k] != src) { stage = c->f[k]; break; }
+    pz_touch(c, stage);
     unsigned int *d_n = (unsigned int *)c->d_small;
     NL_HIP(zero_small(d_n, 4, c->stream));
     {
@@ -2375,6 +2391,7 @@
     else if (!strcmp(key, "last_fsq_min")) *value = c->last_fsq_min;
     else if (!strcmp(key, "last_spec_overflow")) *value = c->last_spec_overflow;
     else if (!strcmp(key, "last_label_sparse")) *value = c->last_label_sparse;
+    else if (!strcmp(key, "prezero_used")) *value = c->prezero_used;
     else if (!strcmp(key, "device_bytes")) *value = (double)nl_ctx_bytes(c->nzl, c->ny, c->nx);
     else if (!strcmp(key, "gauss_yx_max_r")) *value = getenv("NELLIE_NO_FUSED_YX") ? 0 : GM_MAX_R;
     else if (!strcmp(key, "queue_entries")) {
diff --git a/nellie_amd/csrc/nellie_label.hip b/nellie_amd/csrc/nellie_label.hip
--- a/nellie_amd/csrc/nellie_label.hip
+++ b/nellie_amd/csrc/nellie_label.hip
@@ -8,7 +8,7 @@
     NL_ENTER(c);
     if (!host || z0 < 0 || z1 > c->nzl || z0 >= z1) return nl_fail(err, errlen, NL_EINVAL, "bad plane range [%lld,%lld)", (i64)z0, (i64)z1);
     const i64 plane = c->ny * c->nx;
-    c->i_vmax = 3; c->i_gauss = 0; c->i_labels = -1;
+    c->i_vmax = 3; c->i_gauss = 0; c->i_labels = -1; c->prezero_used = 0;
     NL_HIP(hipMemcpyAsync(c->f[c->i_vmax] + z0 * plane, host, (size_t)(z1 - z0) * plane * 4, hipMemcpyHostToDevice, c->stream));
     NL_HIP(hipStreamSynchronize(c->stream));
     c->frangi_ready = 1;
@@ -159,6 +159,7 @@
     i64 gz0 = 0, gnz = 0;
     bool rank_independent_bands = false;
     bool whole_frame_paint = false;
+    bool prezeroed = false;
 };
 static void label_geo_whole(LabelGeo &g) { g.zf_lo = 0; g.zf_hi = (int)g.nz - 1; g.gz0 = 0; g.gnz = g.nz; }
 
@@ -233,10 +234,19 @@
     NL_CHECK_LAUNCH();
     ccl_flatten_kernel<<<gr, 256, 0, c->stream>>>(rs.parent, rs.nruns, rn.p, cap);
     NL_CHECK_LAUNCH();
+    if (lvl2 && g.prezeroed) {
+        rl_fill_u32_kernel<<<gr, 256, 0, c->stream>>>((unsigned int *)link, 0u, rn);
+        NL_CHECK_LAUNCH();
+    }
     return NL_OK;
 }
 
 static int pack_enqueue_fwd(nl_ctx *c, int with_labels, const float *frangi, const int *labels, char *err, size_t errlen);
+static void label_volumes(const nl_ctx *c, const int *out, int idx[3]) {
+    int nf = 0, io = -1;
+    for (int k = 0; k < 4; ++k) if (k != c->i_vmax) { if ((const int *)c->f[k] == out && io < 0) io = k; else idx[nf++] = k; }
+    idx[2] = io >= 0 ? io : idx[2];
+}
 static int number_and_paint(nl_ctx *c, const LabelGeo &g, const RunSet &rs, int *aux, int64_t *n_labels, char *err, size_t errlen,
                             bool *overflow = nullptr) {
     unsigned long long total = 0;
@@ -255,8 +265,12 @@
         NL_HIP(hipMemcpyAsync(c->h_small, d_total, 8, hipMemcpyDeviceToHost, c->stream));
         NL_HIP(hipMemcpyAsync((char *)c->h_small + 8, (unsigned int *)c->d_small + 60, 4, hipMemcpyDeviceToHost, c->stream));
     }
-    rl_paint_kernel<<<grid1d((g.paint_row1 - g.paint_row0) * 64, 256, (i64)1 << 22), 256, 0, c->stream>>>(
-        g.bitsA, rs.row_off, rs.parent, aux, g.paint_out, g.paint_row0, g.paint_row1, g.wpr, (int)g.nx);
+    if (g.prezeroed)
+        rl_paint_kernel<true><<<grid1d((g.paint_row1 - g.paint_row0) * 64, 256, (i64)1 << 22), 256, 0, c->stream>>>(
+            g.bitsA, rs.row_off, rs.parent, aux, g.paint_out, g.paint_row0, g.paint_row1, g.wpr, (int)g.nx);
+    else
+        rl_paint_kernel<false><<<grid1d((g.paint_row1 - g.paint_row0) * 64, 256, (i64)1 << 22), 256, 0, c->stream>>>(
+            g.bitsA, rs.row_off, rs.parent, aux, g.paint_out, g.paint_row0, g.paint_row1, g.wpr, (int)g.nx);
     NL_CHECK_LAUNCH();
     bool packed = false;
     if (c->pack_with_label && g.whole_frame_paint && c->own_lo == 0 && c->own_hi == c->nzl && c->frangi_ready) {
@@ -274,8 +288,8 @@
 
 static int label_core(nl_ctx *c, const LabelGeo &g, int64_t min_area, int fill_holes, int64_t *n_labels, bool *overflow,
                       char *err, size_t errlen) {
-    int free_idx[3], nf = 0;
-    for (int k = 0; k < 4; ++k) if (k != c->i_vmax) free_idx[nf++] = k;
+    int free_idx[3];
+    label_volumes(c, g.paint_out, free_idx);
     const i64 cap = c->n / 2;
     RunSet rs;
     rs.runs = (RunRec *)c->f[free_idx[0]];
@@ -329,12 +343,17 @@
 static int label_out_index(const nl_ctx *c) {
     int last = -1;
     for (int k = 0; k < 4; ++k) if (k != c->i_vmax) last = k;
+    for (int k = 0; k < 4; ++k) if (k != c->i_vmax && pz_is(c, c->f[k])) last = k;
     return last;
 }
 
 extern "C" int nl_label_run(nl_ctx *c, int has_thr, float thr, int64_t min_area, int fill_holes, int64_t *n_labels,
                             char *err, size_t errlen) {
-    NL_ENTER(c);
+    NL_ENTER_KEEP_PZ(c);
+    c->prezero_used &= ~2;
+    const int out_idx = label_out_index(c);
+    const bool pz = pz_is(c, c->f[out_idx]) && c->nzl == c->gnz && !(getenv("NELLIE_LABEL_VOXEL") && atoi(getenv("NELLIE_LABEL_VOXEL"))) && c->nx <= 65535;
+    c->pz_buf = nullptr;
     if (!c->frangi_ready) return nl_fail(err, errlen, NL_ESTATE, "nl_label_run before a Frangi volume exists");
     if (c->nzl != c->gnz) return nl_fail(err, errlen, NL_EINVAL, "nl_label_run works on a whole volume (Z-slabs: nl_label_pack / nl_label_run_global)");
     static int force_voxel = -1;
@@ -345,8 +364,9 @@
     g.nrows = c->nzl * c->ny; g.wpr = (int)((c->nx + 63) / 64); g.nwords = g.nrows * g.wpr;
     g.rows = c->d_rows;
     g.bitsA = (unsigned long long *)c->m[1]; g.bitsB = (unsigned long long *)c->m[2];
-    g.paint_row0 = 0; g.paint_row1 = g.nrows; g.paint_out = (int *)c->f[label_out_index(c)];
+    g.paint_row0 = 0; g.paint_row1 = g.nrows; g.paint_out = (int *)c->f[out_idx];
     g.link_scratch = g.paint_out;
+    g.prezeroed = pz;
     label_geo_whole(g);
     g.whole_frame_paint = true;
     c->pack_pending = 0;
@@ -360,6 +380,7 @@
     int rc = label_core(c, g, min_area, fill_holes, n_labels, &overflow, err, errlen);
     if (rc) return rc;
     if (overflow) return label_run_voxels(c, has_thr, thr, min_area, fill_holes, n_labels, err, errlen);
+    if (pz) c->prezero_used |= 2;
     c->labbits_epoch = c->epoch.load();
     return NL_OK;
 }
@@ -743,7 +764,7 @@
         }
         NL_CHECK_LAUNCH();
     }
-    rl_paint_kernel<<<grid1d((g.paint_row1 - g.paint_row0) * 64, 256, (i64)1 << 22), 256, 0, c->stream>>>(
+    rl_paint_kernel<false><<<grid1d((g.paint_row1 - g.paint_row0) * 64, 256, (i64)1 << 22), 256, 0, c->stream>>>(
         g.bitsA, rs.row_off, rs.parent, sg.aux, g.paint_out, g.paint_row0, g.paint_row1, g.wpr, (int)g.nx);
     NL_CHECK_LAUNCH();
     NL_HIP(hipStreamSynchronize(c->stream));
diff --git a/nellie_amd/csrc/nl_common.h b/nellie_amd/csrc/nl_common.h
--- a/nellie_amd/csrc/nl_common.h
+++ b/nellie_amd/csrc/nl_common.h
@@ -57,6 +57,10 @@
     const unsigned long long *d_support = nullptr;
     unsigned long long labbits_epoch = ~0ull - 8;
     int last_label_sparse = 0;
+    float *pz_buf = nullptr;
+    unsigned long long pz_epoch = ~0ull - 8;
+    int pz_on = 0;
+    int prezero_used = 0;
     unsigned char *mk_act = nullptr; size_t mk_act_cap = 0;
     int mk_act_valid = 0;
     int mk_ntiles = 0;
diff --git a/nellie_amd/csrc/nl_host.h b/nellie_amd/csrc/nl_host.h
--- a/nellie_amd/csrc/nl_host.h
+++ b/nellie_amd/csrc/nl_host.h
@@ -11,6 +11,7 @@
 
 #define NL_MASK_SLOTS 2
 #define NL_VERSION "nellie_amd-hip 0.1.0 (gfx950)"
+#define NL_PREZERO_DEFAULT 1
 #define SCAN_CHUNK 4096
 
 struct CommApi {
@@ -79,6 +80,15 @@
     ++(c)->epoch;                                                      \
     NL_HIP(hipSetDevice((c)->device));
 
+#define NL_ENTER_KEEP_PZ(c)                                            \
+    NL_ENTER(c)                                                        \
+    if ((c)->pz_epoch + 1 == (c)->epoch.load()) (c)->pz_epoch = (c)->epoch.load();
+
+static inline bool pz_valid(const nl_ctx *c) { return c->pz_buf && c->pz_epoch == c->epoch.load(); }
+static inline bool pz_is(const nl_ctx *c, const float *p) { return pz_valid(c) && p == c->pz_buf; }
+static inline void pz_set(nl_ctx *c, float *p) { c->pz_buf = p; c->pz_epoch = c->epoch.load(); }
+static inline void pz_touch(nl_ctx *c, const float *p) { if (p == c->pz_buf) c->pz_buf = nullptr; }
+
 #define NL_ENTER_IO(c)                                                 \
     if (!(c)) return nl_fail(err, errlen, NL_EINVAL, "ctx is NULL");   \
     NL_HIP(hipSetDevice((c)->device));
```

After: 28590 Mvoxel/s, median of 6. 1.1% higher.
